# simon-donike/NIR-GAN

Hardware: AMD Instinct MI355X
Metric: 256x256 RGB tiles/sec (G+D fwd+bwd+step) (higher is better)
Workload: dtype f32 (3xbf16 split, 6 products, f32 accumulate) for the contractions with 32-channel runs incl. the Winograd plane GEMMs; exact f32 MFMA for the first / last layers; f32 everywhere else; 1 GPU; configs[1]: 6-block ResnetGenerator + 3-layer PatchGAN, bs=16/GPU, 256x256, GAN+L1, padding=0, fp32-equivalent MFMA (three bf16 terms, six products); global_batch=16, parallelism=dp1

## Files before the change

### include/nirgan_hip.h

```cpp
#ifndef NIRGAN_HIP_H
#define NIRGAN_HIP_H

#include <stdint.h>

#ifdef __cplusplus
extern "C" {
#endif

#define NIRGAN_MAX_TAPS 16

#define NIRGAN_OK 0
#define NIRGAN_ERR_ARG (-1)
#define NIRGAN_ERR_LAUNCH (-2)

#define NIRGAN_ACT_NONE 0
#define NIRGAN_ACT_RELU 1
#define NIRGAN_ACT_LRELU 2
#define NIRGAN_ACT_TANH 3

#define NIRGAN_BORDER_KEEP 0
#define NIRGAN_BORDER_REFLECT 1

int nirgan_version(void);
const char* nirgan_last_error(void);

typedef struct {
    const float* in;  int64_t in_elems;
    int in_hp, in_wp, in_cs;
    int run;
    int in_stride, in_oh, in_ow;
    int ntaps;
    int tap_dh[NIRGAN_MAX_TAPS], tap_dw[NIRGAN_MAX_TAPS];
    const float* w;   int64_t w_elems;
    const float* bias;
    float* out;       int64_t out_elems;
    int out_hp, out_wp, out_cs;
    int out_stride, out_oh, out_ow;
    int B, OH, OW, N;
    const float* zero_page;
    int ksplit; float* split_ws; int64_t split_ws_elems;
    int precision;
    int w_bf16;
    int in_bf16;
    float* stats_ws; int64_t stats_ws_elems; int stats_chunk0, stats_chunks;
    const float* fuse_y; const float* fuse_mean; const float* fuse_rstd;
    int fuse_h, fuse_w, fuse_oh, fuse_ow, fuse_act; float fuse_slope;
    float* fuse_part; int64_t fuse_part_elems; int fuse_chunk0, fuse_chunks;
    int out_bf16, fuse_y_bf16;
    int algo;
    const void* w_x3; int64_t w_x3_plane;
    int out_span;
} nirgan_conv_desc;
#define NIRGAN_CONV_TILE128 1
#define NIRGAN_CONV_X3_R4 4

int nirgan_conv_igemm(const nirgan_conv_desc* d, void* stream);

typedef struct {
    const float* p;   int64_t p_elems;
    int p_hp, p_wp, p_cs, p_oh, p_ow;
    const float* q;   int64_t q_elems;
    int q_hp, q_wp, q_cs, q_stride, q_oh, q_ow;
    int run, ntaps;
    int tap_dh[NIRGAN_MAX_TAPS], tap_dw[NIRGAN_MAX_TAPS];
    int B, OH, OW, N;
    float* slabs;     int64_t slab_elems;
    int nsplit, rows_per_split;
    const float* zero_page;
    int precision;
    int nplanes; int64_t p_plane, q_plane;
    int pq_bf16;
    int algo;
} nirgan_wgrad_desc;
#define NIRGAN_WGRAD_ONE_UNIT 1
#define NIRGAN_WGRAD_TILE128 2

int nirgan_wgrad_igemm(const nirgan_wgrad_desc* d, void* stream);

int nirgan_conv_igemm_group(const nirgan_conv_desc* const* descs, int n, void* stream);

int nirgan_conv_wgrad_pair(const nirgan_conv_desc* c, const nirgan_wgrad_desc* w, void* stream);

const char* nirgan_conv_kernel_name(const nirgan_conv_desc* d);
const char* nirgan_wgrad_kernel_name(const nirgan_wgrad_desc* d);
const char* nirgan_conv_wgrad_pair_kernel_name(const nirgan_conv_desc* c, const nirgan_wgrad_desc* w);

int nirgan_reduce_rows(const float* slabs, int nsplit, int N, int K, const int32_t* map,
                       float* dst, int64_t dst_elems, int dst_row_stride, int accumulate, void* stream);
int nirgan_reduce_rows_part(const float* slabs, int nsplit, int N, int row0, int rows, int K, const int32_t* map,
                            float* dst, int64_t dst_elems, int dst_row_stride, int accumulate, void* stream);

int nirgan_reduce_rows_batch(const int64_t* jobs_device, int njobs, int total_blocks, void* stream);

int nirgan_pack_rows(const float* src, int64_t src_elems, int src_row_stride, const int32_t* map,
                     float* dst, int N, int K, void* stream);

int nirgan_pack_rows_bf16(const float* src, int64_t src_elems, int src_row_stride, const int32_t* map,
                          void* dst_bf16, int N, int K, void* stream);
int nirgan_pack_rows_batch(const int64_t* jobs_device, int njobs, int total_blocks, void* stream);

int nirgan_split3(const float* src, void* dst_bf16, int64_t n, int64_t plane, void* stream);

typedef struct {
    const float* y;
    int B, H, W, C;
    int norm; float eps;
    float* mean; float* rstd;
    int act; float slope;
    const float* residual; int r_hp, r_wp, r_pad;
    float* out; int o_hp, o_wp, o_pad; int border;
    float* ws; int64_t ws_elems;
    void* out_bf16;
    int stats_chunks;
    const float* stats_shift;
    int y_bf16;
} nirgan_in_fwd_desc;

int64_t nirgan_instnorm_ws_elems(int B, int H, int W, int C);
int nirgan_instnorm_fwd(const nirgan_in_fwd_desc* d, void* stream);

typedef struct {
    const float* g; int g_hp, g_wp, g_pad, g_fold;
    const float* g2;
    const float* a; int a_hp, a_wp, a_pad;
    int act; float slope;
    const float* y; const float* mean; const float* rstd; int norm;
    int B, H, W, C;
    float* dy; int d_hp, d_wp, d_pad;
    float* gsum_out;
    float* dbias;
    float* ws; int64_t ws_elems;
    void* dy_bf16;
    int sums_chunks;
// ... 208 lines not shown
int nirgan_location_encoder(const nirgan_locenc_desc* d, void* stream);

typedef struct {
    const float* image; const float* reference;
    int B, N;
    void* ws; int64_t ws_bytes;
    float* out;
} nirgan_hist_match_desc;

int64_t nirgan_hist_match_ws_bytes(int B, int N);
int nirgan_hist_match(const nirgan_hist_match_desc* d, void* stream);

typedef struct {
    const float* dy; int dy_hp, dy_wp, dy_pad;
    int B, H, W, K;
    float* Yt; int64_t Yt_elems;
    int r;
} nirgan_wino_dy_desc;

typedef struct {
    const float* x; int x_hp, x_wp;
    int B, H, W, C, K;
    const float* U; const float* bias;
    float* V; int64_t V_elems;
    float* M; int64_t M_elems;
    float* y;
    const float* zero_page;
    int r;
    float* stats_ws; int64_t stats_ws_elems;
    const float* fuse_y; const float* fuse_mean; const float* fuse_rstd; const float* fuse_g2;
    float* fuse_gz; float* fuse_part; int64_t fuse_part_elems; int fuse_act; float fuse_slope;
    int algo;
    const void* U3;
} nirgan_wino6_desc;
#define NIRGAN_W6_ONE_TILE 1
#define NIRGAN_W6_DIRECT_TILE 3
#define NIRGAN_W6_X3_R4 5
#define NIRGAN_W6_PATCH_PER_THREAD 16
#define NIRGAN_W6_PATCH_PER_LANES 17
const char* nirgan_wino6_gemm_kernel_name(const nirgan_wino6_desc* d);
const char* nirgan_wino6_pair_kernel_name(const nirgan_wino6_desc* d, const nirgan_wgrad_desc* w);

int64_t nirgan_wino6_tiles(int B, int H, int W);
int64_t nirgan_wino6_tiles_r(int B, int H, int W, int r);
int nirgan_wino6_weights(const float* w, int K, int C, int transpose_flip, float* U, void* stream);
int nirgan_wino6_weights_r(const float* w, int K, int C, int r, int transpose_flip, float* U, void* stream);
int nirgan_wino6_weights_x3(const float* w, int K, int C, int r, int transpose_flip, float* U, void* U3_bf16, void* stream);
int nirgan_wino6_weights_batch(const int64_t* jobs_device, int njobs, int total_blocks, void* stream);
int nirgan_wino6_input(const nirgan_wino6_desc* d, void* stream);
int nirgan_wino6_input_norm(const nirgan_wino6_desc* d, const float* y, const float* mean, const float* rstd, int act, float slope, void* stream);
int nirgan_wino6_gemm(const nirgan_wino6_desc* d, void* stream);
int nirgan_wino6_gemm_wgrad_pair(const nirgan_wino6_desc* c, const nirgan_wgrad_desc* w, void* stream);
int nirgan_wino6_output(const nirgan_wino6_desc* d, void* stream);
int nirgan_wino6_conv3x3(const nirgan_wino6_desc* d, void* stream);
int nirgan_wino6_dy(const nirgan_wino_dy_desc* d, void* stream);
int nirgan_wino6_input_dy(const nirgan_wino6_desc* c, const nirgan_wino_dy_desc* y, void* stream);
int nirgan_wino6_input_dy_norm(const nirgan_wino6_desc* c, const nirgan_wino_dy_desc* y, const nirgan_in_bwd_desc* n, void* stream);
int nirgan_wino6_wgrad_finish(const float* slabs, int nsplit, int K, int C, float* grad, int accumulate, void* stream);
int nirgan_wino6_wgrad_finish_r(const float* slabs, int nsplit, int K, int C, int r, float* grad, int accumulate, void* stream);
int nirgan_wino6_wgrad_finish_batch(const float* const* slabs, float* const* grads, int n, int nsplit, int K, int C, int r, int accumulate, void* stream);

int nirgan_bilinear_fwd(const float* src, int B, int SH, int SW, float* dst, int OH, int OW, void* stream);
int nirgan_bilinear_bwd(const float* ddst, int B, int OH, int OW, float* dsrc, int SH, int SW, void* stream);

typedef struct {
    const float* z; const float* e; const float* scale;
    int style;
    int B, H, W, C;
    float* out; int o_hp, o_wp, o_pad;
} nirgan_inject_fwd_desc;
int nirgan_inject_fwd(const nirgan_inject_fwd_desc* d, void* stream);

typedef struct {
    const float* g; const float* a; int a_hp, a_wp, a_pad;
    const float* z; const float* e; const float* scale;
    int style;
    int B, H, W, C;
    float* dz; float* de; float* dscale;
    float* ws; int64_t ws_elems;
} nirgan_inject_bwd_desc;
int nirgan_inject_bwd(const nirgan_inject_bwd_desc* d, void* stream);

int nirgan_colsum(const float* x, int64_t rows, int cols, float* out, int accumulate, void* stream);

int nirgan_param_scale_fwd(const float* x, const float* param, float* out, int64_t n, void* stream);
int nirgan_param_scale_bwd(const float* gout, const float* x, const float* param, float* gx, float* dparam, float* ws, int64_t ws_elems,
                           int64_t n, void* stream);
int nirgan_fill(float* dst, int64_t n, float value, void* stream);
int nirgan_axpy(float* y, const float* x, int64_t n, float alpha, void* stream);

#define NIRGAN_OP_CONV 1
#define NIRGAN_OP_WGRAD 2
#define NIRGAN_OP_IN_FWD 3
#define NIRGAN_OP_IN_BWD 4
typedef struct { int op; const void* desc; } nirgan_plan_entry;
int nirgan_run_plan(const nirgan_plan_entry* entries, int n, void* stream);

int64_t nirgan_tile_count(int B, int H, int W, int tile, int margin);
int nirgan_tile_gather(const float* scene, int B, int C, int H, int W, int tile, int margin, int first, int n, float* tiles, void* stream);
int nirgan_tile_scatter(const float* tiles, int B, int C, int H, int W, int tile, int margin, int first, int n, float* scene, void* stream);

#define NIRGAN_BLEND_LINEAR 0
#define NIRGAN_BLEND_COSINE 1
typedef struct {
    int B, C, H, W;
    int tile, margin, overlap;
    int window;
    int first, n;
    float* scene;
    float* tiles;
} nirgan_tile_blend_desc;
int64_t nirgan_tile_count_ov(int B, int H, int W, int tile, int margin, int overlap);
int nirgan_tile_gather_ov(const nirgan_tile_blend_desc* d, void* stream);
int nirgan_tile_blend(const nirgan_tile_blend_desc* d, void* stream);

typedef struct {
    int n, C, H, W;
    int views;
    const float* src;
    float* dst;
} nirgan_tile_views_desc;
int nirgan_tile_views_expand(const nirgan_tile_views_desc* d, void* stream);
int nirgan_tile_views_merge(const nirgan_tile_views_desc* d, void* stream);

#define NIRGAN_GEO_SLAB_MAX 2048
typedef struct {
    const double* points;
    int n_points;
    int n_verts;
    const double* verts;
    const int32_t* ring_start;
    const int32_t* ring_region;
    int n_rings, n_regions;
    double* region_box;
    const int32_t* ring_start_host;
    const int32_t* ring_region_host;
    int slab_verts;
    uint32_t* ws;
    int64_t ws_bytes;
    int32_t* region;
} nirgan_point_regions_desc;
int64_t nirgan_point_regions_ws_bytes(int n_points, int n_regions);
int nirgan_region_boxes(const nirgan_point_regions_desc* d, void* stream);
int nirgan_point_regions(const nirgan_point_regions_desc* d, void* stream);

#define NIRGAN_RASTER_U8 0
#define NIRGAN_RASTER_I16 1
#define NIRGAN_RASTER_I32 2
typedef struct {
    const double* points;
    int n_points;
    int H, W, dtype;
    const void* raster;
    double x0, dx, y0, dy;
    int has_nodata, nodata;
    int32_t* value;
} nirgan_raster_lookup_desc;
int nirgan_raster_lookup(const nirgan_raster_lookup_desc* d, void* stream);

#ifdef __cplusplus
}
#endif
#endif
```

### nir-gan_amd/csrc/elementwise.hip

```cpp
#include "common.h"

namespace {

inline int grid_for(int64_t total, int cap = 4096) {
    const int64_t g = (total + 255) / 256;
    return int(g < cap ? (g < 1 ? 1 : g) : cap);
}

__global__ __launch_bounds__(256) void adam_kernel(float* __restrict__ p, const float* __restrict__ g, float* __restrict__ m,
                                                   float* __restrict__ v, int64_t n, float b1, float b2, float eps,
                                                   float step_size, float inv_sqrt_bc2) {
    const int64_t n4 = n >> 2;
    for (int64_t i = blockIdx.x * int64_t(blockDim.x) + threadIdx.x; i < n4; i += int64_t(gridDim.x) * blockDim.x) {
        f32x4 pp = reinterpret_cast<f32x4*>(p)[i];
        const f32x4 gg = reinterpret_cast<const f32x4*>(g)[i];
        f32x4 mm = reinterpret_cast<f32x4*>(m)[i], vv = reinterpret_cast<f32x4*>(v)[i];
#pragma unroll
        for (int k = 0; k < 4; ++k) {
            mm[k] = mm[k] * b1 + (1.f - b1) * gg[k];
            vv[k] = vv[k] * b2 + (1.f - b2) * gg[k] * gg[k];
            const float denom = sqrtf(vv[k]) * inv_sqrt_bc2 + eps;
            pp[k] -= step_size * (mm[k] / denom);
        }
        reinterpret_cast<f32x4*>(p)[i] = pp;
// ... 65 lines not shown
            }
        }
        ds[i] = acc;
    }
}

struct InjP {
    const float* z; const float* e; const float* scale; int style;
    int HW, W, C;
    float* out; int o_row, o_img, o_org;
    const float* g; const float* a; int a_row, a_img, a_org;
    float* dz; float* de; float* dscale; float* ws;
};

__global__ __launch_bounds__(256) void inject_fwd_kernel(const InjP p, int64_t npix) {
    const int q4 = p.C / 4;
    const float s = p.scale ? p.scale[0] : 1.f;
    const int64_t total = npix * q4;
    for (int64_t i = blockIdx.x * int64_t(blockDim.x) + threadIdx.x; i < total; i += int64_t(gridDim.x) * blockDim.x) {
        const int q = int(i % q4);
        const int64_t pix = i / q4;
        const int b = int(pix / p.HW), r = int(pix - int64_t(b) * p.HW);
        const int h = r / p.W, w = r - h * p.W;
        const float ev = p.e[pix];
        f32x4 v = *reinterpret_cast<const f32x4*>(p.z + pix * p.C + q * 4);
        if (p.style == 0) v = v * (p.scale ? 1.f + s * ev : ev); else v = v + s * ev;
#pragma unroll
        for (int k = 0; k < 4; ++k) v[k] = v[k] > 0.f ? v[k] : 0.f;
        *reinterpret_cast<f32x4*>(p.out + int64_t(b) * p.o_img + p.o_org + int64_t(h) * p.o_row + int64_t(w) * p.C + q * 4) = v;
    }
}

__global__ __launch_bounds__(256) void inject_bwd_kernel(const InjP p, int64_t npix) {
    __shared__ float red[256];
    const int q4 = p.C / 4 < 256 ? p.C / 4 : 256;
    const int ppi = 256 / q4;
    const int tid = threadIdx.x, q = tid % q4, pl = tid / q4;
    const float s = p.scale ? p.scale[0] : 1.f;
    float ds_acc = 0.f;
    for (int64_t base = int64_t(blockIdx.x) * ppi; base < npix; base += int64_t(gridDim.x) * ppi) {
        const int64_t pix = base + pl;
        float de_part = 0.f;
        if (pl < ppi && pix < npix) {
            const int b = int(pix / p.HW), r = int(pix - int64_t(b) * p.HW);
            const int h = r / p.W, w = r - h * p.W;
            const float ev = p.e[pix];
            const float mul = p.scale ? 1.f + s * ev : ev;
            for (int qq = q; qq < p.C / 4; qq += q4) {
                const f32x4 gv = *reinterpret_cast<const f32x4*>(p.g + pix * p.C + qq * 4);
                const f32x4 av = *reinterpret_cast<const f32x4*>(p.a + int64_t(b) * p.a_img + p.a_org + int64_t(h) * p.a_row + int64_t(w) * p.C + qq * 4);
                const f32x4 zv = *reinterpret_cast<const f32x4*>(p.z + pix * p.C + qq * 4);
                f32x4 gm, dz;
#pragma unroll
                for (int k = 0; k < 4; ++k) {
                    gm[k] = av[k] > 0.f ? gv[k] : 0.f;
                    if (p.style == 0) {
                        dz[k] = gm[k] * mul;
                        de_part += gm[k] * zv[k] * s;
                        ds_acc += gm[k] * zv[k] * ev;
                    } else {
                        dz[k] = gm[k];
                        de_part += gm[k] * s;
                        ds_acc += gm[k] * ev;
                    }
                }
                *reinterpret_cast<f32x4*>(p.dz + pix * p.C + qq * 4) = dz;
            }
        }
        red[tid] = de_part;
        __syncthreads();
        if (q == 0 && pl < ppi && pix < npix) {
            float t = 0.f;
            for (int k = 0; k < q4; ++k) t += red[pl * q4 + k];
            p.de[pix] = t;
        }
        __syncthreads();
    }
    ds_acc = ng_wave_sum(ds_acc);
    if ((tid & 63) == 0) red[tid >> 6] = ds_acc;
    __syncthreads();
    if (tid == 0 && p.dscale) p.ws[blockIdx.x] = (red[0] + red[1]) + (red[2] + red[3]);
}

__global__ __launch_bounds__(1024) void colsum_kernel(const float* __restrict__ x, int64_t rows, int cols, float* __restrict__ out, int accumulate) {
    __shared__ float red[16][64];
    const int cl = threadIdx.x & 63, c = blockIdx.x * 64 + cl, rl = threadIdx.x >> 6;
    float s0 = 0.f, s1 = 0.f, s2 = 0.f, s3 = 0.f;
    if (c < cols) {
        int64_t r = rl;
        for (; r + 48 < rows; r += 64) {
            s0 += x[r * cols + c];
            s1 += x[(r + 16) * cols + c];
            s2 += x[(r + 32) * cols + c];
            s3 += x[(r + 48) * cols + c];
        }
        for (; r < rows; r += 16) s0 += x[r * cols + c];
    }
    red[rl][cl] = (s0 + s1) + (s2 + s3);
    __syncthreads();
    if (rl == 0 && c < cols) {
        float t = 0.f;
#pragma unroll
        for (int i = 0; i < 16; ++i) t += red[i][cl];
        out[c] = accumulate ? out[c] + t : t;
    }
}

__global__ void fill_kernel(float* __restrict__ dst, int64_t n, float v) {
    for (int64_t i = blockIdx.x * int64_t(blockDim.x) + threadIdx.x; i < n; i += int64_t(gridDim.x) * blockDim.x) dst[i] = v;
}

__global__ void axpy_kernel(float* __restrict__ y, const float* __restrict__ x, int64_t n, float a) {
    for (int64_t i = blockIdx.x * int64_t(blockDim.x) + threadIdx.x; i < n; i += int64_t(gridDim.x) * blockDim.x) y[i] += a * x[i];
}


__global__ __launch_bounds__(256) void param_scale_fwd_kernel(const float* __restrict__ x, const float* __restrict__ param, float* __restrict__ out, int64_t n) {
    const float c = *param;
    for (int64_t i = blockIdx.x * 256ll + threadIdx.x; i < n; i += int64_t(gridDim.x) * 256) out[i] = x[i] * c;
}
__global__ __launch_bounds__(256) void param_scale_bwd_kernel(const float* __restrict__ gout, const float* __restrict__ x, const float* __restrict__ param,
                                                               float* __restrict__ gx, float* __restrict__ ws, int64_t n) {
    __shared__ float red[4];
    const float c = *param;
    float acc = 0.f;
    for (int64_t i = blockIdx.x * 256ll + threadIdx.x; i < n; i += int64_t(gridDim.x) * 256) {
        const float g = gout[i];
        gx[i] = g * c;
        acc += g * x[i];
    }
    acc = ng_wave_sum(acc);
    if ((threadIdx.x & 63) == 0) red[threadIdx.x >> 6] = acc;
    __syncthreads();
    if (threadIdx.x == 0) ws[blockIdx.x] = (red[0] + red[1]) + (red[2] + red[3]);
}

__global__ __launch_bounds__(256) void partials_finish_kernel(const float* __restrict__ ws, int rows, int nv, float* dst) {
    __shared__ float part[4][8];
    const int tid = threadIdx.x, lane = tid & 63, wave = tid >> 6;
    float acc[8] = {0, 0, 0, 0, 0, 0, 0, 0};
    for (int r = tid; r < rows; r += 256)
        for (int i = 0; i < nv; ++i) acc[i] += ws[size_t(r) * nv + i];
    for (int i = 0; i < nv; ++i) {
        const float v = ng_wave_sum(acc[i]);
        if (lane == 0) part[wave][i] = v;
    }
    __syncthreads();
    if (tid < nv) atomicAdd(dst + tid, (part[0][tid] + part[1][tid]) + (part[2][tid] + part[3][tid]));
}

}

int ng_partials_finish(const float* ws, int rows, int nv, float* dst, hipStream_t st) {
    NG_REQUIRE(ws && dst && rows > 0 && nv > 0 && nv <= 8, "partials_finish: bad arguments");
    hipLaunchKernelGGL(partials_finish_kernel, dim3(1), dim3(256), 0, st, ws, rows, nv, dst);
    return nirgan_check_launch("partials_finish");
}

extern "C" int nirgan_adam(float* p, const float* g, float* m, float* v, int64_t n, float lr, float beta1, float beta2,
                           float eps, int step, void* stream) {
    NG_REQUIRE(p && g && m && v && n > 0 && step >= 1, "adam: bad arguments");
    NG_REQUIRE(ng_aligned16(p) && ng_aligned16(g) && ng_aligned16(m) && ng_aligned16(v), "adam: pointers must be 16-byte aligned");
    const double bc1 = 1.0 - pow(double(beta1), double(step));
    const double bc2 = 1.0 - pow(double(beta2), double(step));
    const float step_size = float(double(lr) / bc1);
    const float inv_sqrt_bc2 = float(1.0 / sqrt(bc2));
    hipLaunchKernelGGL(adam_kernel, dim3(grid_for((n + 3) / 4, 2048)), dim3(256), 0, static_cast<hipStream_t>(stream),
                       p, g, m, v, n, beta1, beta2, eps, step_size, inv_sqrt_bc2);
    return nirgan_check_launch("adam");
}

extern "C" int nirgan_bilinear_fwd(const float* src, int B, int SH, int SW, float* dst, int OH, int OW, void* stream) {
    NG_REQUIRE(src && dst && B > 0 && SH > 0 && SW > 0 && OH > 0 && OW > 0, "bilinear_fwd: bad arguments");
    hipLaunchKernelGGL(bilinear_fwd_kernel, dim3(grid_for(int64_t(B) * OH * OW)), dim3(256), 0, static_cast<hipStream_t>(stream), src, B, SH, SW, dst, OH, OW);
    return nirgan_check_launch("bilinear_fwd");
}

extern "C" int nirgan_bilinear_bwd(const float* ddst, int B, int OH, int OW, float* dsrc, int SH, int SW, void* stream) {
    NG_REQUIRE(ddst && dsrc && B > 0 && SH > 0 && SW > 0 && OH > 0 && OW > 0, "bilinear_bwd: bad arguments");
    hipStream_t st = static_cast<hipStream_t>(stream);
    hipLaunchKernelGGL(bilinear_bwd_kernel, dim3(grid_for(int64_t(B) * SH * SW)), dim3(256), 0, st, ddst, B, OH, OW, dsrc, SH, SW);
    return nirgan_check_launch("bilinear_bwd");
}

extern "C" int nirgan_inject_fwd(const nirgan_inject_fwd_desc* d, void* stream) {
    NG_REQUIRE(d && d->z && d->e && d->out, "inject_fwd: null pointer");
    NG_REQUIRE(d->B > 0 && d->H > 0 && d->W > 0 && d->C >= 4 && d->C % 4 == 0, "inject_fwd: bad shape");
    NG_REQUIRE(d->o_hp == d->H + 2 * d->o_pad && d->o_wp == d->W + 2 * d->o_pad, "inject_fwd: output geometry mismatch");
    InjP p = {};
    p.z = d->z; p.e = d->e; p.scale = d->scale; p.style = d->style; p.HW = d->H * d->W; p.W = d->W; p.C = d->C;
    p.out = d->out; p.o_row = d->o_wp * d->C; p.o_img = d->o_hp * p.o_row; p.o_org = d->o_pad * p.o_row + d->o_pad * d->C;
    const int64_t npix = int64_t(d->B) * p.HW;
    hipLaunchKernelGGL(inject_fwd_kernel, dim3(grid_for(npix * (d->C / 4))), dim3(256), 0, static_cast<hipStream_t>(stream), p, npix);
    return nirgan_check_launch("inject_fwd");
}

extern "C" int nirgan_inject_bwd(const nirgan_inject_bwd_desc* d, void* stream) {
    NG_REQUIRE(d && d->g && d->a && d->z && d->e && d->dz && d->de, "inject_bwd: null pointer");
    NG_REQUIRE(d->B > 0 && d->H > 0 && d->W > 0 && d->C >= 4 && d->C % 4 == 0, "inject_bwd: bad shape");
    NG_REQUIRE(d->a_hp == d->H + 2 * d->a_pad && d->a_wp == d->W + 2 * d->a_pad, "inject_bwd: mask geometry mismatch");
    InjP p = {};
    p.z = d->z; p.e = d->e; p.scale = d->scale; p.style = d->style; p.HW = d->H * d->W; p.W = d->W; p.C = d->C;
    p.g = d->g; p.a = d->a; p.a_row = d->a_wp * d->C; p.a_img = d->a_hp * p.a_row; p.a_org = d->a_pad * p.a_row + d->a_pad * d->C;
    p.dz = d->dz; p.de = d->de; p.dscale = d->dscale;
    const int64_t npix = int64_t(d->B) * p.HW;
    const int q4 = d->C / 4 < 256 ? d->C / 4 : 256;
    const int ppi = 256 / q4;
    int64_t g = (npix + ppi - 1) / ppi;
    g = g < 2048 ? g : 2048;
    NG_REQUIRE(!d->dscale || (d->ws && d->ws_elems >= g), "inject_bwd: dscale needs a workspace of %lld floats (block partial sums, fixed-order finish)", (long long)g);
    p.ws = d->ws;
    hipLaunchKernelGGL(inject_bwd_kernel, dim3(int(g)), dim3(256), 0, static_cast<hipStream_t>(stream), p, npix);
    if (d->dscale) return ng_partials_finish(d->ws, int(g), 1, d->dscale, static_cast<hipStream_t>(stream));
    return nirgan_check_launch("inject_bwd");
}

extern "C" int nirgan_param_scale_fwd(const float* x, const float* param, float* out, int64_t n, void* stream) {
    NG_REQUIRE(x && param && out && n > 0, "param_scale_fwd: bad arguments");
    hipLaunchKernelGGL(param_scale_fwd_kernel, dim3(grid_for(n)), dim3(256), 0, static_cast<hipStream_t>(stream), x, param, out, n);
    return nirgan_check_launch("param_scale_fwd");
}

extern "C" int nirgan_param_scale_bwd(const float* gout, const float* x, const float* param, float* gx, float* dparam, float* ws, int64_t ws_elems,
                                      int64_t n, void* stream) {
    NG_REQUIRE(gout && x && param && gx && dparam && ws && n > 0, "param_scale_bwd: bad arguments");
    int64_t g = (n + 255) / 256;
    g = g < 1024 ? g : 1024;
    NG_REQUIRE(ws_elems >= g, "param_scale_bwd: workspace holds %lld floats, %lld needed", (long long)ws_elems, (long long)g);
    hipLaunchKernelGGL(param_scale_bwd_kernel, dim3(int(g)), dim3(256), 0, static_cast<hipStream_t>(stream), gout, x, param, gx, ws, n);
    return ng_partials_finish(ws, int(g), 1, dparam, static_cast<hipStream_t>(stream));
}

extern "C" int nirgan_colsum(const float* x, int64_t rows, int cols, float* out, int accumulate, void* stream) {
    NG_REQUIRE(x && out && rows > 0 && cols > 0, "colsum: bad arguments");
    hipLaunchKernelGGL(colsum_kernel, dim3((cols + 63) / 64), dim3(1024), 0, static_cast<hipStream_t>(stream), x, rows, cols, out, accumulate);
    return nirgan_check_launch("colsum");
}

extern "C" int nirgan_fill(float* dst, int64_t n, float value, void* stream) {
    NG_REQUIRE(dst && n > 0, "fill: bad arguments");
    hipLaunchKernelGGL(fill_kernel, dim3(grid_for(n)), dim3(256), 0, static_cast<hipStream_t>(stream), dst, n, value);
    return nirgan_check_launch("fill");
}

extern "C" int nirgan_axpy(float* y, const float* x, int64_t n, float alpha, void* stream) {
    NG_REQUIRE(y && x && n > 0, "axpy: bad arguments");
    hipLaunchKernelGGL(axpy_kernel, dim3(grid_for(n)), dim3(256), 0, static_cast<hipStream_t>(stream), y, x, n, alpha);
    return nirgan_check_launch("axpy");
}

extern "C" int nirgan_run_plan(const nirgan_plan_entry* entries, int n, void* stream) {
    NG_REQUIRE(entries || n == 0, "run_plan: null entries");
    for (int i = 0; i < n; ++i) {
        int rc;
        switch (entries[i].op) {
            case NIRGAN_OP_CONV: rc = nirgan_conv_igemm(static_cast<const nirgan_conv_desc*>(entries[i].desc), stream); break;
            case NIRGAN_OP_WGRAD: rc = nirgan_wgrad_igemm(static_cast<const nirgan_wgrad_desc*>(entries[i].desc), stream); break;
            case NIRGAN_OP_IN_FWD: rc = nirgan_instnorm_fwd(static_cast<const nirgan_in_fwd_desc*>(entries[i].desc), stream); break;
            case NIRGAN_OP_IN_BWD: rc = nirgan_instnorm_bwd(static_cast<const nirgan_in_bwd_desc*>(entries[i].desc), stream); break;
            default: nirgan_set_error("run_plan: unknown op %d at entry %d", entries[i].op, i); return NIRGAN_ERR_ARG;
        }
        if (rc != NIRGAN_OK) return rc;
    }
    return NIRGAN_OK;
}
```

### nir-gan_amd/csrc/igemm_conv.hip

```cpp
#include "igemm_tiles.h"
#include "igemm_tile256.h"
#include "igemm_x3.h"
#include <cstdlib>
#include "igemm_x3r.h"

namespace {

template <int BN, int PREC = 0, bool WB16 = false, bool AB16 = false>
__global__ __launch_bounds__(256, 2) void conv_igemm_kernel(const ng::ConvParams p) {
    __shared__ __attribute__((aligned(16))) char st0[(128 + BN) * 128];
    __shared__ __attribute__((aligned(16))) char st1[(128 + BN) * 128];
    ng::conv_tile<BN, PREC, WB16, AB16>(p, blockIdx.x, st0, st1);
}

__global__ __launch_bounds__(512, 2) void conv_igemm256_kernel(const ng::ConvParams p) {
    __shared__ __attribute__((aligned(16))) char lds[ng::T256_LDS];
    ng::conv_tile256(p, ng_xcd_remap(blockIdx.x, gridDim.x), lds);
}

template <int BN>
__global__ __launch_bounds__(512, 2) void conv_x3_kernel(const ng::X3Work w) {
    __shared__ __attribute__((aligned(16))) char sA0[ng::X3_A_BYTES];
    __shared__ __attribute__((aligned(16))) char sA1[ng::X3_A_BYTES];
    __shared__ __attribute__((aligned(16))) char sB0[3 * BN * 64];
// ... 47 lines not shown
__global__ __launch_bounds__(256, 2) void conv_group_kernel(const ConvGroup g) {
    __shared__ __attribute__((aligned(16))) char st0[(128 + BN) * 128];
    __shared__ __attribute__((aligned(16))) char st1[(128 + BN) * 128];
    const int bid = blockIdx.x;
    int k = 0;
    if (bid >= g.first[1]) k = 1;
    if (bid >= g.first[2]) k = 2;
    if (bid >= g.first[3]) k = 3;
    if (k == 0) ng::conv_tile<BN, PREC, WB16, AB16>(g.p[0], bid, st0, st1);
    else if (k == 1) ng::conv_tile<BN, PREC, WB16, AB16>(g.p[1], bid - g.first[1], st0, st1);
    else if (k == 2) ng::conv_tile<BN, PREC, WB16, AB16>(g.p[2], bid - g.first[2], st0, st1);
    else ng::conv_tile<BN, PREC, WB16, AB16>(g.p[3], bid - g.first[3], st0, st1);
}

}

int ng::ng_cu_count_conv() {
    static int cus = 0;
    if (cus == 0) {
        int dev = 0, n = 0;
        if (hipGetDevice(&dev) != hipSuccess || hipDeviceGetAttribute(&n, hipDeviceAttributeMultiprocessorCount, dev) != hipSuccess || n <= 0) n = 256;
        cus = n;
#ifdef NG_X3R_STAMP
        if (const char* e = getenv("NG_X3R_CUS")) cus = atoi(e);
#endif
    }
    return cus;
}
using ng::ng_cu_count_conv;

int ng::ng_launch_conv_x3(const ng::ConvParams* ps, const int n, const int bn, const int nplanes, const long long in_plane, const long long w3_pstride,
                          const long long out_plane, hipStream_t st, const char* what) {
    ng::X3Work w;
    int total = 0;
    for (int i = 0; i < n; ++i) { w.p[i] = ps[i]; w.first[i] = total; total += ng::conv_x3_tiles(ps[i], bn) * (nplanes > 1 ? nplanes : 1); }
    for (int i = n; i < 4; ++i) { w.p[i] = ps[0]; w.first[i] = 0x7fffffff; }
    w.first[n] = total;
    for (int i = n + 1; i < 5; ++i) w.first[i] = 0x7fffffff;
    w.n = n;
    w.nplanes = nplanes > 1 ? nplanes : 1;
    w.in_plane = in_plane; w.w3_pstride = w3_pstride; w.out_plane = out_plane;
    w.spread = 0;
    for (int i = 0; i < 4; ++i) w.start[i] = 0;
    const int G = ng_cu_count_conv();
    bool unequal = false;
    for (int i = 1; i < n; ++i) unequal = unequal || ps[i].K != ps[0].K;
    if (n >= 2 && w.nplanes == 1 && unequal && total >= G && G <= 1024) {
        long long load[2 * 1024 + 1];
        for (int i = 0; i < G; ++i) load[i] = 0;
        int order[4] = {0, 1, 2, 3};
        for (int i = 0; i < n; ++i)
            for (int j = i + 1; j < n; ++j)
                if (ps[order[j]].K > ps[order[i]].K) { const int t = order[i]; order[i] = order[j]; order[j] = t; }
        for (int oi = 0; oi < n; ++oi) {
            const int k = order[oi];
            const int rem = (w.first[k + 1] - w.first[k]) % G;
            if (rem == 0) continue;
            const long long cost = ps[k].K / 32 + 3;
            long long prefix[2 * 1024 + 1];
            prefix[0] = 0;
            for (int i = 0; i < 2 * G; ++i) prefix[i + 1] = prefix[i] + load[i % G];
            int best = 0;
            for (int s0 = 1; s0 < G; ++s0)
                if (prefix[s0 + rem] - prefix[s0] < prefix[best + rem] - prefix[best]) best = s0;
            for (int t = 0; t < rem; ++t) load[(best + t) % G] += cost;
            w.start[k] = best;
        }
        w.spread = 1;
    }
    const dim3 grid(total < G ? total : G);
    switch (ng::conv_x3_route(ps, n, bn)) {
        case ng::X3R_GENERIC: hipLaunchKernelGGL((conv_x3r_kernel<128, 2>), grid, dim3(256), 0, st, w); break;
        case ng::X3R_STATS: hipLaunchKernelGGL((conv_x3r_kernel<128, 1>), grid, dim3(256), 0, st, w); break;
        case ng::X3R_PLAIN: hipLaunchKernelGGL((conv_x3r_kernel<128, 0>), grid, dim3(256), 0, st, w); break;
        case ng::X3_N128: hipLaunchKernelGGL(conv_x3_kernel<128>, grid, dim3(512), 0, st, w); break;
        case ng::X3_N64: hipLaunchKernelGGL(conv_x3_kernel<64>, grid, dim3(512), 0, st, w); break;
    }
    return nirgan_check_launch(what);
}

ng::X3Kernel ng::conv_x3_route(const ng::ConvParams* ps, const int n, const int bn) {
    bool reg_fed = true, gen = false, stats = false;
    for (int i = 0; i < n; ++i) {
        reg_fed = reg_fed && ng::conv_x3r_ok(ps[i], bn);
        gen = gen || ng::conv_x3r_generic(ps[i]);
        stats = stats || ng::conv_x3r_stats(ps[i]);
    }
    if (reg_fed) return gen ? ng::X3R_GENERIC : (stats ? ng::X3R_STATS : ng::X3R_PLAIN);
    return bn == 128 ? ng::X3_N128 : ng::X3_N64;
}

enum ConvKernel { CONV_K_X3R, CONV_K_X3_N128, CONV_K_X3_N64, CONV_K_TILE256, CONV_K_TILE128, CONV_K_TILE64 };
static const char* const CONV_KERNEL_NAMES[] = {"conv_x3r_kernel<128>", "conv_x3_kernel<128>", "conv_x3_kernel<64>", "conv_igemm256_kernel",
                                                "conv_igemm_kernel<128>", "conv_igemm_kernel<64>"};
struct ConvRoute { ConvKernel k; int bn; };
static ConvRoute conv_route(const ng::ConvParams* ps, const int n, const bool group) {
    bool x3 = ps[0].prec == 3;
    for (int i = 0; i < n; ++i) x3 = x3 && ng::conv_x3_ok(ps[i]) && (ps[i].N % 128 == 0) == (ps[0].N % 128 == 0);
    if (x3) {
        const int bn = ng::conv_x3_bn(ps, n, ng_cu_count_conv());
        const ng::X3Kernel k = ng::conv_x3_route(ps, n, bn);
        return {k == ng::X3_N128 ? CONV_K_X3_N128 : (k == ng::X3_N64 ? CONV_K_X3_N64 : CONV_K_X3R), bn};
    }
    if (!group && ps[0].algo != NIRGAN_CONV_TILE128 && ng::conv_tile256_ok(ps[0])) return {CONV_K_TILE256, 0};
    return {ps[0].N > 64 ? CONV_K_TILE128 : CONV_K_TILE64, 0};
}
static bool conv_route_x3(const ConvRoute& r) { return r.k == CONV_K_X3R || r.k == CONV_K_X3_N128 || r.k == CONV_K_X3_N64; }

#ifdef NG_X3R_STAMP
extern "C" int nirgan_x3r_stamps(unsigned long long* host, int n) {
    return hipMemcpyFromSymbol(host, HIP_SYMBOL(ng::ng_x3r_stamps), size_t(n) * 8) == hipSuccess ? 0 : -1;
}
#endif

extern "C" int nirgan_split3(const float* src, void* dst_bf16, int64_t n, int64_t plane, void* stream) {
    NG_REQUIRE(src && dst_bf16 && n > 0 && n % 8 == 0 && plane >= n && plane % 8 == 0, "split3: n and plane must be positive multiples of 8, plane >= n");
    NG_REQUIRE(ng_aligned16(src) && ng_aligned16(dst_bf16), "split3: pointers must be 16-byte aligned");
    hipLaunchKernelGGL(split3_kernel, dim3((unsigned)((n / 8 + 255) / 256)), dim3(256), 0, static_cast<hipStream_t>(stream),
                       src, static_cast<unsigned short*>(dst_bf16), (long long)n, (long long)plane);
    return nirgan_check_launch("split3");
}

extern "C" int nirgan_conv_igemm(const nirgan_conv_desc* d, void* stream) {
    ng::ConvParams p;
    const int rc = ng::build_conv_params(d, p);
    if (rc != NIRGAN_OK) return rc;
    hipStream_t st = static_cast<hipStream_t>(stream);
    const ConvRoute r = conv_route(&p, 1, false);
    if (conv_route_x3(r)) return ng::ng_launch_conv_x3(&p, 1, r.bn, 1, 0, 0, 0, st, "conv_igemm (three-term split tile)");
    if (p.prec == 3) {
        NG_REQUIRE(p.ch == p.N, "conv: out_span = 2 needs a problem the three-term split tile covers (run %% 32 == 0, N %% 64 == 0)");
        p.prec = 0;
    }
    if (r.k == CONV_K_TILE256) {
        hipLaunchKernelGGL(conv_igemm256_kernel, dim3(((p.M + 255) >> 8) * (p.N >> 8)), dim3(512), 0, st, p);
        return nirgan_check_launch("conv_igemm (256 x 256 tile)");
    }
    const dim3 grid(p.mtiles * p.ntiles * p.ksplit);
    ng::conv_tile_form(p, [&](auto form) {
        using F = decltype(form);
        if (r.k == CONV_K_TILE128) hipLaunchKernelGGL((conv_igemm_kernel<128, F::prec, F::wb16, F::ab16>), grid, dim3(256), 0, st, p);
        else hipLaunchKernelGGL((conv_igemm_kernel<64, F::prec, F::wb16, F::ab16>), grid, dim3(256), 0, st, p);
    });
    if (p.ksplit > 1) {
        const long long total = (long long)p.M * (p.N / 4);
        const int grid = int((total + 255) / 256 < 4096 ? (total + 255) / 256 : 4096);
        hipLaunchKernelGGL(conv_splitk_reduce_kernel, dim3(grid), dim3(256), 0, st, p);
    }
    return nirgan_check_launch("conv_igemm");
}

extern "C" const char* nirgan_conv_kernel_name(const nirgan_conv_desc* d) {
    ng::ConvParams p;
    if (ng::build_conv_params(d, p) != NIRGAN_OK) return nullptr;
    return CONV_KERNEL_NAMES[conv_route(&p, 1, false).k];
}

extern "C" int nirgan_conv_igemm_group(const nirgan_conv_desc* const* descs, int n, void* stream) {
    NG_REQUIRE(descs != nullptr && n >= 1 && n <= 4, "conv_igemm_group: 1..4 descriptors");
    ConvGroup g;
    int total = 0;
    bool wide = false;
    for (int i = 0; i < n; ++i) {
        NG_REQUIRE(descs[i] != nullptr, "conv_igemm_group: null descriptor %d", i);
        const int rc = ng::build_conv_params(descs[i], g.p[i]);
        if (rc != NIRGAN_OK) return rc;
        NG_REQUIRE(descs[i]->ksplit <= 1, "conv_igemm_group: split-K descriptors are not groupable");
// ... 27 lines not shown
```

### nir-gan_amd/csrc/igemm_tiles.h

```cpp
#pragma once
#include <type_traits>
#include "common.h"

#ifdef NG_DIAG
__device__ __forceinline__ unsigned long long ng_stamp() {
    unsigned long long t;
    __builtin_amdgcn_sched_barrier(0);
    asm volatile("s_memtime %0\n\ts_waitcnt lgkmcnt(0)" : "=s"(t) :: "memory");
    __builtin_amdgcn_sched_barrier(0);
    return t;
}
#define NG_DIAG_ENTRY const unsigned long long ng_entry = ng_stamp();
#define NG_DIAG_DECL unsigned long long ng_t0 = ng_stamp(), ng_a = ng_t0, ng_wait = 0, ng_body = 0, ng_b = 0;
#define NG_WAIT_BEGIN ng_a = ng_stamp();
#define NG_WAIT_END ng_b = ng_stamp(); ng_wait += ng_b - ng_a; ng_a = ng_b;
#define NG_BODY_END ng_b = ng_stamp(); ng_body += ng_b - ng_a; ng_a = ng_b;
#define NG_DIAG_STORE(dbg, blk)                                                                          \
    if ((threadIdx.x & 63) == 0 && (dbg) != nullptr) {                                                     \
        unsigned long long* o = (dbg) + (size_t(blk) * 4 + (threadIdx.x >> 6)) * 6;                         \
        const unsigned long long te = ng_stamp();                                                           \
        o[0] = ng_t0; o[1] = ng_loop_end; o[2] = te; o[3] = ng_wait; o[4] = ng_body;                        \
        o[5] = ng_t0 - ng_entry;                               \
    }
#else
#define NG_DIAG_ENTRY
#define NG_DIAG_DECL
#define NG_WAIT_BEGIN
#define NG_WAIT_END
#define NG_BODY_END
#define NG_DIAG_STORE(dbg, blk)
#endif

namespace ng {

typedef __bf16 bf16x8 __attribute__((ext_vector_type(8)));
typedef float f32x8 __attribute__((ext_vector_type(8)));

__device__ __forceinline__ bf16x8 ng_bf16_round(const f32x8 v) { return __builtin_convertvector(v, bf16x8); }
__device__ __forceinline__ f32x8 ng_bf16_widen(const bf16x8 v) { return __builtin_convertvector(v, f32x8); }

template <int PREC>
__device__ __forceinline__ void ng_mfma_bf16(const f32x8 a, const f32x8 b, f32x16& acc) {
    const bf16x8 ah = ng_bf16_round(a), bh = ng_bf16_round(b);
    if constexpr (PREC == 2) {
        const bf16x8 am = ng_bf16_round(a - ng_bf16_widen(ah)), bm = ng_bf16_round(b - ng_bf16_widen(bh));
        acc = __builtin_amdgcn_mfma_f32_32x32x16_bf16(am, bh, acc, 0, 0, 0);
        acc = __builtin_amdgcn_mfma_f32_32x32x16_bf16(ah, bm, acc, 0, 0, 0);
    }
    acc = __builtin_amdgcn_mfma_f32_32x32x16_bf16(ah, bh, acc, 0, 0, 0);
}

struct ConvParams {
    const float* in;
    const float* w;
    const float* bias;
    float* out;
    const float* zero;
    int in_row, in_img, in_cs, run, in_stride, in_org;
    int ntaps;
    int tap_off[NIRGAN_MAX_TAPS];
    int K;
    int out_cs, out_row, out_img, out_stride, out_org;
    int OW, OHW, M, N;
    int mtiles, ntiles;
    int ksplit;
    float* split_ws;
    unsigned long long* dbg;
    int w_bf16;
    int in_bf16;
    int prec;
    float* stats;
    int stats_chunk0, stats_cps;
    const float* f_y; const float* f_mean; const float* f_rstd; float* f_part;
    int f_img, f_row, f_org, f_act, f_chunk0, f_cps;
    float f_slope;
    int out16, f_y16;
    int algo;
    int off32;
    const unsigned short* w3;
    long long w3_plane;
    int ch;
    long long out_elems;
};


template <int BN, int PREC, bool WB16 = false, bool AB16 = false>
__device__ __forceinline__ void conv_tile(const ConvParams& p, const int block_id, char* st0, char* st1,
                                          const float* in_base = nullptr, const float* w_base = nullptr, float* out_base = nullptr) {
    NG_DIAG_ENTRY
    const float* const p_in = in_base ? in_base : p.in;
    const float* const p_w = w_base ? w_base : p.w;
    float* const p_out = out_base ? out_base : p.out;
    static_assert(!WB16 || PREC == 1, "bf16-stored weights are consumed by the bf16 operand mode only");
    static_assert(!AB16 || WB16, "bf16 activations come with bf16-stored weights");
    constexpr int BM = 128;
    constexpr int A_BYTES = BM * 128;
    constexpr int B_BYTES = BN * 128;
    constexpr int STAGE = A_BYTES + B_BYTES;
    constexpr int NT = BN / 64;
    constexpr int BI = BN / 32;
    constexpr bool WIDE = AB16;
    constexpr int KS = WIDE ? 64 : 32;

    const int tid = threadIdx.x, lane = tid & 63;
    const int wave = __builtin_amdgcn_readfirstlane(tid >> 6);
    const int tiles = p.mtiles * p.ntiles;
    const int rid = ng_xcd_remap(block_id, tiles * p.ksplit);
    const int ksp = rid / tiles, id = rid - ksp * tiles;
    const int n0 = (id % p.ntiles) * BN, m0 = (id / p.ntiles) * BM;

    const int lrow = lane >> 3, lchunk = lane & 7;
    constexpr int AIW = 4;
    int a_base[AIW], a_col[AIW];
#pragma unroll
    for (int i = 0; i < AIW; ++i) {
        const int row = (wave * 4 + i) * 8 + lrow;
        const int lc = lchunk ^ ((row >> 1) & 7);
        const int cw = AB16 ? 8 : 4;
        int m = m0 + row;
        m = m < p.M ? m : p.M - 1;
        const int b = m / p.OHW, r = m - b * p.OHW;
        const int oh = r / p.OW, ow = r - oh * p.OW;
        a_col[i] = lc * cw;
        a_base[i] = b * p.in_img + oh * p.in_stride * p.in_row + ow * p.in_stride * p.in_cs + p.in_org + lc * cw;
    }
    constexpr int BIW = (WB16 && !WIDE) ? BN / 64 : BI;
    int b_base[BIW], b_col[BIW];
    bool b_ok[BIW];
#pragma unroll
    for (int i = 0; i < BIW; ++i) {
        if constexpr (WIDE) {
            const int row = (wave * BI + i) * 8 + lrow;
            const int lc = lchunk ^ ((row >> 1) & 7);
            const int n = n0 + row;
            b_ok[i] = n < p.N;
            b_col[i] = lc * 8;
            b_base[i] = (b_ok[i] ? n : 0) * p.K + lc * 8;
        } else if constexpr (WB16) {
            const int row = (wave * BIW + i) * 16 + (lane >> 2);
            const int lc = (lane & 3) ^ ((row >> 2) & 3);
            const int n = n0 + row;
            b_ok[i] = n < p.N;
            b_col[i] = lc * 8;
            b_base[i] = (b_ok[i] ? n : 0) * p.K + lc * 8;
        } else {
            const int row = (wave * BI + i) * 8 + lrow;
            const int lc = lchunk ^ ((row >> 1) & 7);
            const int n = n0 + row;
            b_ok[i] = n < p.N;
            b_col[i] = lc * 4;
            b_base[i] = (b_ok[i] ? n : 0) * p.K + lc * 4;
        }
    }

    constexpr int ESA = AB16 ? 2 : 4, ESB = WB16 ? 2 : 4;
    unsigned a_boff[AIW], b_boff[BIW];
#pragma unroll
    for (int i = 0; i < AIW; ++i) a_boff[i] = unsigned(a_base[i]) * unsigned(ESA);
#pragma unroll
    for (int i = 0; i < BIW; ++i) b_boff[i] = unsigned(b_base[i]) * unsigned(ESB);
    const bool inside = p.off32 != 0;

    auto issue = [&](char* sA, int t, int c0) {
        char* sB = sA + A_BYTES;
        const int toff = p.tap_off[t] + c0;
// ... 210 lines not shown
    }

#ifdef NG_DIAG
    const unsigned long long ng_loop_end = ng_stamp();
#endif
#ifdef NG_DIAG_SKIP_EPILOGUE
    if (p.dbg == nullptr) {
        float keep = 0.f;
#pragma unroll
        for (int mt = 0; mt < 2; ++mt)
#pragma unroll
            for (int nt = 0; nt < NT; ++nt)
#pragma unroll
                for (int r = 0; r < 16; ++r) keep += acc[mt][nt][r];
        if (keep == 123456.789f) p_out[0] = keep;
        return;
    }
#endif
    if (p.stats != nullptr) {
        const int b = m0 / p.OHW;
        const int chunk = p.stats_chunk0 + ((m0 - b * p.OHW) >> 7) * 2 + wr;
        float* sp = p.stats + (size_t(b) * p.stats_cps + chunk) * 4 * p.N;
#pragma unroll
        for (int nt = 0; nt < NT; ++nt) {
            const float own = acc[0][nt][0], other = __shfl_xor(own, 32, 64);
            const float k = half == 0 ? own : other;
            float s1 = 0.f, s2 = 0.f;
#pragma unroll
            for (int mt = 0; mt < 2; ++mt)
#pragma unroll
                for (int r = 0; r < 16; ++r) {
                    const float v = acc[mt][nt][r] - k;
                    s1 += v;
                    s2 += v * v;
                }
            s1 += __shfl_xor(s1, 32, 64);
            s2 += __shfl_xor(s2, 32, 64);
            const int col = n0 + wc * (BN / 2) + nt * 32 + (lane & 31);
            if (half == 0 && col < p.N) {
                sp[col] = k;
                sp[p.N + col] = s1;
                sp[2 * p.N + col] = s2;
                sp[3 * p.N + col] = 64.f;
            }
        }
    }
    __syncthreads();
    {
        float* half_base = reinterpret_cast<float*>(wr == 0 ? st0 : st1);
#pragma unroll
        for (int mt = 0; mt < 2; ++mt)
#pragma unroll
            for (int nt = 0; nt < NT; ++nt) {
                const int col = wc * (BN / 2) + nt * 32 + (lane & 31);
#pragma unroll
                for (int r = 0; r < 16; ++r) {
                    const int row_l = mt * 32 + (r & 3) + 8 * (r >> 2) + 4 * half;
                    half_base[row_l * BN + col] = acc[mt][nt][r];
                }
            }
    }
    __syncthreads();
    auto write_out = [&](auto wtag) {
        constexpr int W = decltype(wtag)::value;
        constexpr int LPR = BN / W;
        constexpr int RPP = 256 / LPR;
        typedef float fW __attribute__((ext_vector_type(W)));
        typedef __bf16 bW __attribute__((ext_vector_type(W)));
        const int chunk = tid % LPR, row0 = tid / LPR;
        const int n = n0 + chunk * W;
        fW bv = {};
        const bool to_ws = p.ksplit > 1;
        if (p.bias != nullptr && !to_ws) {
#pragma unroll
            for (int j = 0; j < W; ++j) bv[j] = n + j < p.N ? p.bias[n + j] : 0.f;
        }
        int m = m0 + row0;
        const int mc = m < p.M ? m : p.M - 1;
        int b = mc / p.OHW;
        const int r0 = mc - b * p.OHW;
        int oh = r0 / p.OW, ow = r0 - oh * p.OW;
        const int OH = p.OHW / p.OW;
        const bool fused = p.f_y != nullptr;
        const int fb = m0 / p.OHW;
        fW fm = {}, fr = {}, s1 = {}, s2 = {};
        if (fused && n < p.N) {
            fm = *reinterpret_cast<const fW*>(p.f_mean + size_t(fb) * p.N + n);
            fr = *reinterpret_cast<const fW*>(p.f_rstd + size_t(fb) * p.N + n);
        }
        const float fneg = p.f_act == NIRGAN_ACT_RELU ? 0.f : (p.f_act == NIRGAN_ACT_LRELU ? p.f_slope : 1.f);
#pragma unroll 4
        for (int row = row0; row < BM; row += RPP) {
            if (m < p.M && n < p.N) {
                const float* src = reinterpret_cast<const float*>(row < 64 ? st0 : st1) + (row & 63) * BN + chunk * W;
                fW v = *reinterpret_cast<const fW*>(src);
                v += bv;
                const int oidx = b * p.out_img + oh * p.out_stride * p.out_row + ow * p.out_stride * p.out_cs + p.out_org + n;
                float* dst = to_ws ? p.split_ws + ((size_t(ksp) * p.M + m) * p.N + n) : p_out + oidx;
                if constexpr (W == 8) {
                    *reinterpret_cast<bW*>(reinterpret_cast<unsigned short*>(p_out) + oidx) = __builtin_convertvector(v, bW);
                } else if (p.out16) {
                    *reinterpret_cast<bW*>(reinterpret_cast<unsigned short*>(p_out) + oidx) = __builtin_convertvector(v, bW);
                } else if (n + 4 <= p.N) {
                    *reinterpret_cast<fW*>(dst) = v;
                } else {
#pragma unroll
                    for (int j = 0; j < W; ++j)
                        if (n + j < p.N) dst[j] = v[j];
                }
                if (fused) {
                    const size_t yidx = size_t(b) * p.f_img + size_t(oh * p.out_stride) * p.f_row + size_t(ow * p.out_stride) * p.N + p.f_org + n;
                    fW y4;
                    if (p.f_y16) y4 = __builtin_convertvector(*reinterpret_cast<const bW*>(reinterpret_cast<const unsigned short*>(p.f_y) + yidx), fW);
                    else y4 = *reinterpret_cast<const fW*>(p.f_y + yidx);
                    const fW z = (y4 - fm) * fr;
#pragma unroll
                    for (int j = 0; j < W; ++j) {
                        const float gz = z[j] > 0.f ? v[j] : v[j] * fneg;
                        s1[j] += gz;
                        s2[j] += gz * z[j];
                    }
                }
            }
            m += RPP;
            ow += RPP;
            while (ow >= p.OW) { ow -= p.OW; ++oh; }
            while (oh >= OH) { oh -= OH; ++b; }
        }
        if (fused) {
            __syncthreads();
            fW* red = reinterpret_cast<fW*>(st0);
            red[tid * 2] = s1;
            red[tid * 2 + 1] = s2;
            __syncthreads();
            if (tid < LPR && n < p.N) {
                fW t1 = {}, t2 = {};
#pragma unroll 4
                for (int r = 0; r < RPP; ++r) {
                    t1 += red[(r * LPR + tid) * 2];
                    t2 += red[(r * LPR + tid) * 2 + 1];
                }
                float* pp = p.f_part + (size_t(fb) * p.f_cps + p.f_chunk0 + ((m0 - fb * p.OHW) >> 7)) * 2 * p.N + n;
                *reinterpret_cast<fW*>(pp) = t1;
                *reinterpret_cast<fW*>(pp + p.N) = t2;
            }
        }
    };
    if (p.out16 && p.N % BN == 0 && p.ksplit <= 1 && ((p.out_cs | p.out_org | p.out_row | p.out_img) & 7) == 0) write_out(std::integral_constant<int, 8>{});
    else write_out(std::integral_constant<int, 4>{});
    NG_DIAG_STORE(p.dbg, block_id)
}

struct WgradParams {
    const float* p;
    const float* q;
    float* slabs;
    const float* zero;
    int p_row, p_img, p_cs, p_org;
    int q_row, q_img, q_cs, q_stride, q_org;
    int run, ntaps;
    int tap_off[NIRGAN_MAX_TAPS];
    int K, OW, OH, OHW, M, N;
    int rows_per_split, nsplit, ntiles_n, ntiles_k;
    int prec;
    int pq_bf16;
    int nplanes;
    long long p_plane, q_plane;
    unsigned long long* dbg;
    int fast32_bytes;
    int fast32;
};


template <int TN, int PREC>
__device__ __forceinline__ void wgrad_tile(const WgradParams& p, const int block_id, char* st0, char* st1) {
    constexpr int P_BYTES = 32 * TN * 4;
    constexpr int Q_BYTES = 32 * 128 * 4;
    constexpr int STAGE = P_BYTES + Q_BYTES;
    constexpr int LPR = TN / 4;
    constexpr int RPI = 64 / LPR;
    constexpr int PI = TN / 32;
    constexpr int EA = TN / 64;

    const int tid = threadIdx.x, lane = tid & 63;
    const int wave = __builtin_amdgcn_readfirstlane(tid >> 6);
    const int tiles = p.ntiles_n * p.ntiles_k;
    const int per_plane = tiles * p.nsplit;
    const int rid = ng_xcd_remap(block_id, per_plane * p.nplanes);
    const int plane = rid / per_plane, id = rid - plane * per_plane;
    const int split = id / tiles, tile = id - split * tiles;
    const int n0 = (tile % p.ntiles_n) * TN, j0 = (tile / p.ntiles_n) * 128;
    const int mstart = split * p.rows_per_split;
    int mend = mstart + p.rows_per_split;
    mend = mend < p.M ? mend : p.M;
    const int nk = mend > mstart ? (mend - mstart + 31) >> 5 : 0;
// ... 605 lines not shown
template <int P, bool WB, bool AB> struct TileForm { static constexpr int prec = P; static constexpr bool wb16 = WB, ab16 = AB; };
template <class F> inline void conv_tile_form(const ConvParams& p, F&& f) {
    if (p.prec == 0) f(TileForm<0, false, false>{});
    else if (p.prec == 1 && p.in_bf16) f(TileForm<1, true, true>{});
    else if (p.prec == 1 && p.w_bf16) f(TileForm<1, true, false>{});
    else if (p.prec == 1) f(TileForm<1, false, false>{});
    else f(TileForm<2, false, false>{});
}

inline int build_conv_params(const nirgan_conv_desc* d, ConvParams& p) {
    NG_REQUIRE(d != nullptr, "conv: null descriptor");
    NG_REQUIRE(d->in && d->w && d->out && d->zero_page, "conv: null pointer");
    NG_REQUIRE(ng_aligned16(d->in) && ng_aligned16(d->w) && ng_aligned16(d->zero_page) && ng_aligned16(d->out), "conv: in/w/out/zero_page must be 16-byte aligned");
    NG_REQUIRE(d->out_cs % 4 == 0 || d->N < 4, "conv: out_cs must be a multiple of 4");
    NG_REQUIRE(d->B > 0 && d->OH > 0 && d->OW > 0 && d->N > 0, "conv: empty problem B=%d OH=%d OW=%d N=%d", d->B, d->OH, d->OW, d->N);
    NG_REQUIRE(d->ntaps >= 1 && d->ntaps <= NIRGAN_MAX_TAPS, "conv: ntaps=%d out of range", d->ntaps);
    NG_REQUIRE(d->run > 0 && d->run % 4 == 0 && d->in_cs > 0 && d->in_cs % 4 == 0, "conv: run=%d and in_cs=%d must be positive multiples of 4", d->run, d->in_cs);
    NG_REQUIRE(d->in_stride >= 1 && d->out_stride >= 1, "conv: strides must be >= 1");
    NG_REQUIRE(d->in_elems < (int64_t(1) << 31) && d->out_elems < (int64_t(1) << 31) && d->w_elems < (int64_t(1) << 31), "conv: buffers must be < 2^31 floats");
    NG_REQUIRE(d->in_elems >= int64_t(d->B) * d->in_hp * d->in_wp * d->in_cs, "conv: in_elems too small");
    NG_REQUIRE(d->out_elems >= int64_t(d->B) * d->out_hp * d->out_wp * d->out_cs, "conv: out_elems too small");
    NG_REQUIRE(d->w_elems >= int64_t(d->N) * d->ntaps * d->run, "conv: w_elems too small");
    const int span = d->out_span > 1 ? d->out_span : 1;
    const bool span_view = span == 2 && d->out_cs == d->N;
    NG_REQUIRE(span == 1 || (span == 2 && d->precision == 3 && d->N % 8 == 0 && (span_view ? d->fuse_y == nullptr : (d->out_cs == d->N / 2 && d->out_stride >= 2))
                             && !d->out_bf16 && !d->fuse_y_bf16 && d->ksplit <= 1 && d->w_x3 != nullptr),
               "conv: out_span=%d needs precision 3 with its weight planes, out_cs == N / 2 and out_stride >= 2 (or out_cs == N), fp32 tensors and no split-K", d->out_span);
    const int ch = d->N / span;
    NG_REQUIRE(ch <= d->out_cs, "conv: %d channels per pixel exceed out_cs=%d", ch, d->out_cs);
    int dh0 = d->tap_dh[0], dh1 = d->tap_dh[0], dw0 = d->tap_dw[0], dw1 = d->tap_dw[0];
    for (int t = 1; t < d->ntaps; ++t) {
        dh0 = d->tap_dh[t] < dh0 ? d->tap_dh[t] : dh0; dh1 = d->tap_dh[t] > dh1 ? d->tap_dh[t] : dh1;
        dw0 = d->tap_dw[t] < dw0 ? d->tap_dw[t] : dw0; dw1 = d->tap_dw[t] > dw1 ? d->tap_dw[t] : dw1;
    }
    NG_REQUIRE(d->in_oh + dh0 >= 0 && (d->OH - 1) * d->in_stride + d->in_oh + dh1 < d->in_hp, "conv: input rows out of range");
    NG_REQUIRE(d->in_ow + dw0 >= 0 && int64_t((d->OW - 1) * d->in_stride + d->in_ow + dw1) * d->in_cs + d->run <= int64_t(d->in_wp) * d->in_cs, "conv: input columns out of range");
    NG_REQUIRE(d->out_oh >= 0 && (d->OH - 1) * d->out_stride + d->out_oh < d->out_hp && d->out_ow >= 0 && (d->OW - 1) * d->out_stride + d->out_ow + (span_view ? 0 : span - 1) < d->out_wp, "conv: output window out of range");

    p.in = d->in; p.w = d->w; p.bias = d->bias; p.out = d->out; p.zero = d->zero_page;
    p.in_cs = d->in_cs; p.in_row = d->in_wp * d->in_cs; p.in_img = d->in_hp * p.in_row;
    p.run = d->run; p.in_stride = d->in_stride; p.in_org = d->in_oh * p.in_row + d->in_ow * d->in_cs;
    p.ntaps = d->ntaps;
    for (int t = 0; t < NIRGAN_MAX_TAPS; ++t) p.tap_off[t] = t < d->ntaps ? d->tap_dh[t] * p.in_row + d->tap_dw[t] * d->in_cs : 0;
    p.K = d->ntaps * d->run;
    p.out_elems = d->out_elems;
    p.out_cs = d->out_cs; p.out_row = d->out_wp * d->out_cs; p.out_img = d->out_hp * p.out_row;
    p.out_stride = d->out_stride; p.out_org = d->out_oh * p.out_row + d->out_ow * d->out_cs;
    p.OW = d->OW; p.OHW = d->OH * d->OW;
    const int64_t M = int64_t(d->B) * p.OHW;
    NG_REQUIRE(M < (int64_t(1) << 31), "conv: too many output pixels");
    p.M = int(M); p.N = d->N; p.ch = ch;
    p.mtiles = (p.M + 127) / 128;
    p.ntiles = d->N > 64 ? (d->N + 127) / 128 : 1;
    NG_REQUIRE(d->precision >= 0 && d->precision <= 3, "conv: precision=%d (0 fp32, 1 bf16, 2 bf16x3, 3 fp32 as three bf16 terms)", d->precision);
    p.prec = d->precision;
    p.w3 = static_cast<const unsigned short*>(d->w_x3);
    p.w3_plane = d->w_x3_plane;
    NG_REQUIRE(p.w3 == nullptr || (ng_aligned16(p.w3) && d->w_x3_plane >= int64_t(d->N) * d->ntaps * d->run && d->w_x3_plane % 8 == 0), "conv: w_x3 misaligned or w_x3_plane too small");
    p.w_bf16 = d->w_bf16 ? 1 : 0;
    NG_REQUIRE(!p.w_bf16 || (d->precision == 1 && d->run % 8 == 0), "conv: bf16-stored weights need precision 1 and run %% 8 == 0 (run=%d)", d->run);
    p.in_bf16 = d->in_bf16 ? 1 : 0;
    NG_REQUIRE(!p.in_bf16 || (p.w_bf16 && d->in_cs % 8 == 0), "conv: bf16 activations need bf16-stored weights and in_cs %% 8 == 0 (in_cs=%d)", d->in_cs);
    p.off32 = (d->in_elems * (p.in_bf16 ? 2 : 4) < (int64_t(1) << 32) && d->w_elems * (p.w_bf16 ? 2 : 4) < (int64_t(1) << 32)) ? 1 : 0;
    NG_REQUIRE(d->algo == 0 || d->algo == NIRGAN_CONV_TILE128 || d->algo == NIRGAN_CONV_X3_R4,
               "conv: algo=%d (0, NIRGAN_CONV_TILE128 or NIRGAN_CONV_X3_R4)", d->algo);
    p.algo = d->algo;
    p.dbg = nullptr;
    p.ksplit = 1;
    p.split_ws = nullptr;
    p.out16 = d->out_bf16 ? 1 : 0;
    p.f_y16 = d->fuse_y_bf16 ? 1 : 0;
    NG_REQUIRE(!p.out16 || (d->N % 4 == 0 && d->out_cs % 4 == 0 && d->ksplit <= 1), "conv: a bf16 output needs N %% 4 == 0, out_cs %% 4 == 0 and no split-K (N=%d)", d->N);
    p.stats = nullptr; p.stats_chunk0 = 0; p.stats_cps = 0;
    if (d->stats_ws != nullptr) {
        NG_REQUIRE(d->ksplit <= 1 && p.OHW % 128 == 0, "conv: the instance-norm partial sums need OH*OW %% 128 == 0 and no split-K (OH*OW=%d)", p.OHW);
        NG_REQUIRE(d->stats_chunk0 >= 0 && d->stats_chunk0 + p.OHW / 64 * span <= d->stats_chunks, "conv: stats_chunk0 + OH*OW/64 (x out_span) exceeds stats_chunks");
        NG_REQUIRE(d->stats_ws_elems >= int64_t(d->B) * d->stats_chunks * 4 * ch, "conv: stats_ws too small (B * stats_chunks * 4 * channels floats)");
        p.stats = d->stats_ws; p.stats_chunk0 = d->stats_chunk0; p.stats_cps = d->stats_chunks;
    }
    p.f_y = nullptr; p.f_mean = nullptr; p.f_rstd = nullptr; p.f_part = nullptr;
    p.f_img = p.f_row = p.f_org = p.f_chunk0 = p.f_cps = 0; p.f_act = NIRGAN_ACT_NONE; p.f_slope = 0.f;
    if (d->fuse_y != nullptr) {
        NG_REQUIRE(d->ksplit <= 1 && p.OHW % 128 == 0 && d->N % 4 == 0 && d->bias == nullptr, "conv: the fused instance-norm backward sums need OH*OW %% 128 == 0, N %% 4 == 0, no split-K and no bias (OH*OW=%d N=%d)", p.OHW, d->N);
        NG_REQUIRE(d->fuse_mean && d->fuse_rstd && d->fuse_part && ng_aligned16(d->fuse_y) && ng_aligned16(d->fuse_mean) && ng_aligned16(d->fuse_rstd) && ng_aligned16(d->fuse_part), "conv: fuse_mean / fuse_rstd / fuse_part missing or misaligned");
        NG_REQUIRE(d->fuse_oh >= 0 && d->fuse_ow >= 0 && (d->OH - 1) * d->out_stride + d->fuse_oh < d->fuse_h && (d->OW - 1) * d->out_stride + d->fuse_ow + span - 1 < d->fuse_w, "conv: fused window out of y's %d x %d extent", d->fuse_h, d->fuse_w);
        NG_REQUIRE(int64_t(d->B) * d->fuse_h * d->fuse_w * ch < (int64_t(1) << 31), "conv: fuse_y must be < 2^31 floats");
        NG_REQUIRE(d->fuse_chunk0 >= 0 && d->fuse_chunk0 + p.OHW / 128 * span <= d->fuse_chunks, "conv: fuse_chunk0 + OH*OW/128 (x out_span) exceeds fuse_chunks");
        NG_REQUIRE(d->fuse_part_elems >= int64_t(d->B) * d->fuse_chunks * 2 * ch, "conv: fuse_part too small");
        NG_REQUIRE(d->fuse_act == NIRGAN_ACT_NONE || d->fuse_act == NIRGAN_ACT_RELU || d->fuse_act == NIRGAN_ACT_LRELU, "conv: fuse_act=%d", d->fuse_act);
        p.f_y = d->fuse_y; p.f_mean = d->fuse_mean; p.f_rstd = d->fuse_rstd; p.f_part = d->fuse_part;
        p.f_row = d->fuse_w * ch; p.f_img = d->fuse_h * p.f_row; p.f_org = d->fuse_oh * p.f_row + d->fuse_ow * ch;
        p.f_act = d->fuse_act; p.f_slope = d->fuse_slope; p.f_chunk0 = d->fuse_chunk0; p.f_cps = d->fuse_chunks;
    }
    if (d->ksplit > 1) {
        const int nk = d->ntaps * ((d->run + 31) / 32);
        NG_REQUIRE(d->split_ws != nullptr && ng_aligned16(d->split_ws), "conv: split_ws missing or misaligned");
        NG_REQUIRE(d->N % 4 == 0, "conv: split-K needs N %% 4 == 0");
        NG_REQUIRE(d->split_ws_elems >= int64_t(d->ksplit) * M * d->N, "conv: split_ws too small");
        const int per = (nk + d->ksplit - 1) / d->ksplit;
        NG_REQUIRE(per * (d->ksplit - 1) < nk, "conv: ksplit=%d too large for %d K-steps", d->ksplit, nk);
        p.ksplit = d->ksplit;
        p.split_ws = d->split_ws;
    }
    return NIRGAN_OK;
}

inline int build_wgrad_params(const nirgan_wgrad_desc* d, WgradParams& p) {
    NG_REQUIRE(d != nullptr, "wgrad_igemm: null descriptor");
    NG_REQUIRE(d->p && d->q && d->slabs && d->zero_page, "wgrad_igemm: null pointer");
    NG_REQUIRE(ng_aligned16(d->p) && ng_aligned16(d->q) && ng_aligned16(d->slabs) && ng_aligned16(d->zero_page), "wgrad_igemm: pointers must be 16-byte aligned");
    NG_REQUIRE(d->B > 0 && d->OH > 0 && d->OW > 0 && d->N > 0, "wgrad_igemm: empty problem");
    NG_REQUIRE(d->p_cs % 4 == 0 && d->q_cs % 4 == 0 && d->run % 4 == 0 && d->run > 0, "wgrad_igemm: p_cs, q_cs, run must be multiples of 4");
    NG_REQUIRE(d->ntaps >= 1 && d->ntaps <= NIRGAN_MAX_TAPS, "wgrad_igemm: ntaps=%d out of range", d->ntaps);
    NG_REQUIRE(d->q_stride >= 1, "wgrad_igemm: q_stride must be >= 1");
    NG_REQUIRE(d->p_elems < (int64_t(1) << 31) && d->q_elems < (int64_t(1) << 31), "wgrad_igemm: buffers must be < 2^31 floats");
    NG_REQUIRE(d->p_elems >= int64_t(d->B) * d->p_hp * d->p_wp * d->p_cs, "wgrad_igemm: p_elems too small");
    NG_REQUIRE(d->q_elems >= int64_t(d->B) * d->q_hp * d->q_wp * d->q_cs, "wgrad_igemm: q_elems too small");
    NG_REQUIRE(((d->N + 3) & ~3) <= d->p_cs, "wgrad_igemm: N (rounded up to 4) exceeds p_cs");
    NG_REQUIRE(d->p_oh >= 0 && d->OH - 1 + d->p_oh < d->p_hp && d->p_ow >= 0 && d->OW - 1 + d->p_ow < d->p_wp, "wgrad_igemm: p window out of range");
    int dh0 = d->tap_dh[0], dh1 = d->tap_dh[0], dw0 = d->tap_dw[0], dw1 = d->tap_dw[0];
    for (int t = 1; t < d->ntaps; ++t) {
        dh0 = d->tap_dh[t] < dh0 ? d->tap_dh[t] : dh0; dh1 = d->tap_dh[t] > dh1 ? d->tap_dh[t] : dh1;
        dw0 = d->tap_dw[t] < dw0 ? d->tap_dw[t] : dw0; dw1 = d->tap_dw[t] > dw1 ? d->tap_dw[t] : dw1;
    }
    NG_REQUIRE(d->q_oh + dh0 >= 0 && (d->OH - 1) * d->q_stride + d->q_oh + dh1 < d->q_hp, "wgrad_igemm: q rows out of range");
    NG_REQUIRE(d->q_ow + dw0 >= 0 && int64_t((d->OW - 1) * d->q_stride + d->q_ow + dw1) * d->q_cs + d->run <= int64_t(d->q_wp) * d->q_cs, "wgrad_igemm: q columns out of range");
    const int64_t M = int64_t(d->B) * d->OH * d->OW;
    NG_REQUIRE(M < (int64_t(1) << 31), "wgrad_igemm: too many pixels");
    NG_REQUIRE(d->nsplit >= 1 && d->rows_per_split > 0 && d->rows_per_split % 32 == 0 && int64_t(d->nsplit) * d->rows_per_split >= M, "wgrad_igemm: bad split (nsplit=%d rows=%d M=%lld)", d->nsplit, d->rows_per_split, (long long)M);
    const int K = d->ntaps * d->run;
    NG_REQUIRE(d->slab_elems >= int64_t(d->nsplit) * d->N * K, "wgrad_igemm: slab_elems too small");

    p.p = d->p; p.q = d->q; p.slabs = d->slabs; p.zero = d->zero_page;
    p.p_cs = d->p_cs; p.p_row = d->p_wp * d->p_cs; p.p_img = d->p_hp * p.p_row; p.p_org = d->p_oh * p.p_row + d->p_ow * d->p_cs;
    p.q_cs = d->q_cs; p.q_row = d->q_wp * d->q_cs; p.q_img = d->q_hp * p.q_row; p.q_stride = d->q_stride;
    p.q_org = d->q_oh * p.q_row + d->q_ow * d->q_cs;
    p.run = d->run; p.ntaps = d->ntaps;
    for (int t = 0; t < NIRGAN_MAX_TAPS; ++t) p.tap_off[t] = t < d->ntaps ? d->tap_dh[t] * p.q_row + d->tap_dw[t] * d->q_cs : 0;
    p.K = K; p.OW = d->OW; p.OH = d->OH; p.OHW = d->OH * d->OW; p.M = int(M); p.N = d->N;
    p.rows_per_split = d->rows_per_split; p.nsplit = d->nsplit;
    p.ntiles_k = (K + 127) / 128;
    p.ntiles_n = d->N > 64 ? (d->N + 127) / 128 : 1;
    NG_REQUIRE(d->precision >= 0 && d->precision <= 3, "wgrad_igemm: precision=%d (0 fp32, 1 bf16, 2 bf16x3, 3 fp32 as three bf16 terms)", d->precision);
    NG_REQUIRE(d->algo == 0 || d->algo == NIRGAN_WGRAD_ONE_UNIT || d->algo == NIRGAN_WGRAD_TILE128,
               "wgrad_igemm: algo=%d (0, NIRGAN_WGRAD_ONE_UNIT or NIRGAN_WGRAD_TILE128)", d->algo);
    p.prec = d->precision;
    p.nplanes = d->nplanes > 1 ? d->nplanes : 1;
    p.p_plane = d->p_plane; p.q_plane = d->q_plane;
    NG_REQUIRE(p.nplanes == 1 || ((d->precision == 0 || d->precision == 3) && !d->pq_bf16 && d->p_plane > 0 && d->q_plane > 0), "wgrad_igemm: planes need the fp32 tile and positive plane strides");
    NG_REQUIRE(d->slab_elems >= int64_t(p.nplanes) * d->nsplit * d->N * K, "wgrad_igemm: slab_elems too small for %d planes", p.nplanes);
    NG_REQUIRE(d->p_elems >= (p.nplanes - 1) * d->p_plane + int64_t(d->B) * d->p_hp * d->p_wp * d->p_cs && d->q_elems >= (p.nplanes - 1) * d->q_plane + int64_t(d->B) * d->q_hp * d->q_wp * d->q_cs, "wgrad_igemm: p/q too small for the planes");
    p.pq_bf16 = d->pq_bf16 ? 1 : 0;
    p.dbg = nullptr;
    {
        bool taps_ok = true;
        for (int t = 0; t < d->ntaps; ++t) taps_ok = taps_ok && (d->tap_dh[t] * p.q_row + d->tap_dw[t] * d->q_cs >= 0);
        const int ms = d->pq_bf16 ? 64 : 32, es = d->pq_bf16 ? 2 : 4;
        p.fast32_bytes = (d->p_elems * es < (int64_t(1) << 32) && d->q_elems * es < (int64_t(1) << 32)) ? 1 : 0;
        p.fast32 = (taps_ok && d->OW % ms == 0 && p.M % ms == 0 && d->rows_per_split % ms == 0
                    && d->p_elems * es < (int64_t(1) << 32) && d->q_elems * es < (int64_t(1) << 32)) ? 1 : 0;
    }
    NG_REQUIRE(!p.pq_bf16 || (d->precision == 1 && d->N > 64 && d->N % 8 == 0 && d->run % 8 == 0 && d->p_cs % 8 == 0 && d->q_cs % 8 == 0),
               "wgrad_igemm: bf16 twins need precision 1, N > 64 and N, run, p_cs, q_cs multiples of 8");
    return NIRGAN_OK;
}

}
```

### nir-gan_amd/csrc/igemm_x3.h

```cpp
#pragma once
#include "igemm_tiles.h"

namespace ng {

constexpr int X3_A_TERM = 256 * 64;
constexpr int X3_A_BYTES = 3 * X3_A_TERM;

__device__ __forceinline__ int x3_key(const int row) { return (0x78 >> (2 * ((row >> 2) & 3))) & 3; }

__device__ __forceinline__ f32x4 ng_gld16_so(const char* base, unsigned off) {
    asm volatile("" : "+v"(off));
    return *reinterpret_cast<const NG_GLOBAL f32x4*>((const NG_GLOBAL char*)base + off);
}

typedef __bf16 bf16x2 __attribute__((ext_vector_type(2)));
typedef unsigned u32x4 __attribute__((ext_vector_type(4)));
__device__ __forceinline__ unsigned x3_pk(const float a, const float b) {
    const f32x2 v = {a, b};
    return __builtin_bit_cast(unsigned, __builtin_convertvector(v, bf16x2));
}
__device__ __forceinline__ float x3_sub(const float a, const float b) {
    float r;
    asm("v_sub_f32 %0, %1, %2" : "=v"(r) : "v"(a), "v"(b));
    return r;
// ... 187 lines not shown
            X3_RB(bad, 3) X3_WAIT(3) mma(0, A[0], 2); __builtin_amdgcn_sched_barrier(0);
            X3_RA(A[1], aad, 1) X3_WAIT(3) mma(0, A[0], 3); __builtin_amdgcn_sched_barrier(0);
        } else {
            X3_RB(bad, 1) X3_WAIT(3) mma(0, A[0], 0); __builtin_amdgcn_sched_barrier(0);
            X3_RA(A[1], aad, 1) X3_WAIT(3) mma(0, A[0], 1); __builtin_amdgcn_sched_barrier(0);
        }
        X3_RA(A[0], aad, 2) X3_WAIT(3)
#pragma unroll
        for (int nt = 0; nt < NT; ++nt) mma(1, A[1], nt);
        __builtin_amdgcn_sched_barrier(0);
        X3_RA(A[1], aad, 3) X3_WAIT(3)
        mid(0);
#pragma unroll
        for (int nt = 0; nt < NT; ++nt) mma(2, A[0], nt);
        __builtin_amdgcn_sched_barrier(0);
        if constexpr (MORE) { X3_WAIT(3) } else { X3_WAIT(0) }
        mid(1);
#pragma unroll
        for (int nt = 0; nt < NT; ++nt) mma(3, A[1], nt);
    };
#undef X3_WAIT
#undef X3_RB
#undef X3_RA
#undef X3_DSR
    constexpr int ESTORES = 2 * (32 / (64 / (CW / 4)));
    auto step = [&](const int cur, char* nA, char* nB, const bool more, const bool behind_stores = false) {
        if (behind_stores) {
            if constexpr (ESTORES == 16) asm volatile("s_waitcnt vmcnt(16)" ::: "memory");
            else asm volatile("s_waitcnt vmcnt(8)" ::: "memory");
        } else {
            asm volatile("s_waitcnt vmcnt(0)" ::: "memory");
        }
        __syncthreads();
        const unsigned aad = cur == 0 ? a_ad0 : a_ad1, bad = cur == 0 ? b_ad0 : b_ad1;
        if (more) {
            compute(aad, bad, std::true_type{}, [&]() { issueB(nB); loadA(); advance(); }, [&](const int j) { commitA(nA, j); });
        } else {
            compute(aad, bad, std::false_type{}, []() {}, [](const int) {});
        }
    };

    auto epilogue = [&]() -> bool {
        const NG_CONST ConvParams& p = *E.p;
        const int pM = p.M, pN = p.N, OHW = p.OHW, OW = p.OW, OH = p.OHW / p.OW, out_img = p.out_img, out_row = p.out_row * p.out_stride,
                  out_px = p.out_cs * p.out_stride, out_org = p.out_org, f_img = p.f_img, f_row = p.f_row * p.out_stride, f_px = p.ch * p.out_stride,
                  f_org = p.f_org, pC = p.ch, span = p.N / p.ch;
        const float* const f_y = p.f_y;
        const int mbase = E.m0 + wr * 64;
        const bool full = E.m0 + 256 <= pM;
        if (p.stats != nullptr && mbase < pM) {
            const int b = mbase / OHW;
            float* sp = p.stats + (size_t(b) * p.stats_cps + p.stats_chunk0 + ((mbase - b * OHW) >> 6) * span) * 4 * pC;
#pragma unroll
            for (int nt = 0; nt < NT; ++nt) {
                const float k0 = __shfl(acc[0][nt][0], lane & 15, 64);
                float s1 = 0.f, s2 = 0.f;
#pragma unroll
                for (int mt = 0; mt < 4; ++mt)
#pragma unroll
                    for (int r = 0; r < 4; ++r) {
                        const float v = acc[mt][nt][r] - k0;
                        s1 += v;
                        s2 += v * v;
                    }
                s1 += __shfl_xor(s1, 16, 64);
                s2 += __shfl_xor(s2, 16, 64);
                s1 += __shfl_xor(s1, 32, 64);
                s2 += __shfl_xor(s2, 32, 64);
                int col = E.n0 + wc * CW + nt * 16 + (lane & 15);
                if (col >= pC) col += 3 * pC;
                if (lane < 16) {
                    sp[col] = k0;
                    sp[pC + col] = s1;
                    sp[2 * pC + col] = s2;
                    sp[3 * pC + col] = 64.f;
                }
            }
        }
        constexpr int LPR = CW / 4, RPP = 64 / LPR;
        constexpr int SWM = CW / 16 - 1;
        const int sw_wr = ((lane >> 4) & SWM) << 4;
        float* const stg = reinterpret_cast<float*>(wave < 6 ? sA1 + wave * 8192 : sB1 + (wave - 6) * 8192);
        const bool fused = f_y != nullptr;
        const float fneg = p.f_act == NIRGAN_ACT_RELU ? 0.f : (p.f_act == NIRGAN_ACT_LRELU ? p.f_slope : 1.f);
        const int chunk = lane % LPR, lrow = lane / LPR;
        const int n = E.n0 + wc * CW + chunk * 4;
        f32x4 bv = {0.f, 0.f, 0.f, 0.f};
        if (p.bias != nullptr) bv = *reinterpret_cast<const f32x4*>(p.bias + n);
        int m = mbase + lrow;
        const int mc = m < pM ? m : pM - 1;
        int b = mc / OHW;
        const int r0 = mc - b * OHW;
        int oh = r0 / OW, ow = r0 - oh * OW;
        const int fb = (mbase < pM ? mbase : pM - 1) / OHW;
        f32x4 fm = {0.f, 0.f, 0.f, 0.f}, fr = fm, s1 = fm, s2 = fm;
        const int nq = n >= pC ? 1 : 0, nc = n - nq * pC;
        if (fused) {
            fm = *reinterpret_cast<const f32x4*>(p.f_mean + size_t(fb) * pC + nc);
            fr = *reinterpret_cast<const f32x4*>(p.f_rstd + size_t(fb) * pC + nc);
        }
        auto halves = [&](auto full_tag) {
            constexpr bool FULL = decltype(full_tag)::value;
            constexpr int P = 32 / RPP;
#pragma unroll
            for (int h = 0; h < 2; ++h) {
#pragma unroll
                for (int q = 0; q < 2; ++q)
#pragma unroll
                    for (int nt = 0; nt < NT; ++nt)
#pragma unroll
                        for (int r = 0; r < 4; ++r) stg[(q * 16 + (lane >> 4) * 4 + r) * CW + ((nt * 16 + (lane & 15)) ^ sw_wr)] = acc[h * 2 + q][nt][r];
                int ooff[P];
                bool ok[P];
                f32x4 yv[P];
#pragma unroll
                for (int pass = 0; pass < P; ++pass) {
                    ok[pass] = FULL || m < pM;
                    ooff[pass] = b * out_img + oh * out_row + ow * out_px + out_org + n;
                    if (fused && ok[pass]) yv[pass] = *reinterpret_cast<const f32x4*>(f_y + (size_t(b) * f_img + size_t(oh) * f_row + size_t(ow) * f_px + f_org + n));
                    m += RPP;
                    ow += RPP;
                    while (ow >= OW) { ow -= OW; ++oh; }
                    while (oh >= OH) { oh -= OH; ++b; }
                }
#pragma unroll
                for (int pass = 0; pass < P; ++pass) {
                    if (ok[pass]) {
                        f32x4 v = *reinterpret_cast<const f32x4*>(stg + (pass * RPP + lrow) * CW + ((chunk * 4) ^ ((((pass * RPP + lrow) >> 2) & SWM) << 4)));
                        v += bv;
#ifdef NG_X3_NT_STORES
                        __builtin_nontemporal_store(v, reinterpret_cast<f32x4*>(E.out + ooff[pass]));
#else
                        *reinterpret_cast<f32x4*>(E.out + ooff[pass]) = v;
#endif
                        if (fused) {
                            const f32x4 z = (yv[pass] - fm) * fr;
#pragma unroll
                            for (int q = 0; q < 4; ++q) {
                                const float gz = z[q] > 0.f ? v[q] : v[q] * fneg;
                                s1[q] += gz;
                                s2[q] += gz * z[q];
                            }
                        }
                    }
                }
            }
        };
        if (full) halves(std::true_type{}); else halves(std::false_type{});
        if (fused) {
#pragma unroll
            for (int q = 0; q < 4; ++q)
#pragma unroll
                for (int o = LPR; o < 64; o <<= 1) {
                    s1[q] += __shfl_xor(s1[q], o, 64);
                    s2[q] += __shfl_xor(s2[q], o, 64);
                }
            f32x4* const red = reinterpret_cast<f32x4*>(sRed);
            if (lane < LPR) {
                red[(wave * LPR + chunk) * 2] = s1;
                red[(wave * LPR + chunk) * 2 + 1] = s2;
            }
            __syncthreads();
            if ((wr & 1) == 0 && lane < LPR && mbase < pM) {
                const f32x4 t1 = s1 + red[((wave + 2) * LPR + chunk) * 2], t2 = s2 + red[((wave + 2) * LPR + chunk) * 2 + 1];
                float* pp = p.f_part + (size_t(fb) * p.f_cps + p.f_chunk0 + ((mbase - fb * OHW) >> 7) * span + nq) * 2 * pC + nc;
                *reinterpret_cast<f32x4*>(pp) = t1;
                *reinterpret_cast<f32x4*>(pp + pC) = t2;
            }
            __syncthreads();
        }
        return full;
    };

    int item = blockIdx.x;
    if (item >= total) return;
    locate(item, L);
    if (L.nk < 0) return;
    begin();
    loadA();
    issueB(sB0);
    advance();
    commitA(sA0, 0);
    commitA(sA0, 1);
    bool behind = false;
    while (true) {
        zero();
        const int nk = L.nk;
        int k = 0;
        if (nk >= 2) {
            if (behind) step(0, sA1, sB1, true, true); else step(0, sA1, sB1, true);
            step(1, sA0, sB0, 2 < nk);
            k = 2;
        }
        for (; k + 2 <= nk; k += 2) {
            step(0, sA1, sB1, true);
            step(1, sA0, sB0, k + 2 < nk);
        }
        if (k < nk) step(0, sA1, sB1, false);
        E = L;
        item += G;
        bool more = wp->spread ? true : item < total;
        __syncthreads();
        if (more) {
            locate(item, L);
            more = L.nk >= 0;
        }
        if (more) {
            begin();
            loadA();
            issueB(sB0);
            advance();
        }
        behind = epilogue();
        if (!more) break;
        commitA(sA0, 0);
        commitA(sA0, 1);
    }
}
// ... 227 lines not shown
```

### nir-gan_amd/nirgan_hip/engine.py

```python
from __future__ import annotations

import ctypes as C
from typing import Dict, List, Optional

import numpy as np
import torch

from . import geometry as G
from . import lib as L
from .options import OPT

IN_EPS = 1e-5


def _ptr(t: Optional[torch.Tensor]) -> Optional[int]:
    return None if t is None else t.data_ptr()


PRECISIONS = {"fp32": 0, "bf16": 1, "bf16x3": 2}


def precision_code(precision) -> int:
    if precision in PRECISIONS.values():
        return int(precision)
# ... 188 lines not shown
        self.ctx = ctx
        self.cache: Dict[tuple, torch.Tensor] = {}

    def packed(self, plan: Plan, param: torch.Tensor, spec: G.PackSpec, rows_alloc: Optional[int] = None, fp32: bool = False) -> torch.Tensor:
        key = (param.data_ptr(), spec.key, fp32)
        if key in self.cache:
            return self.cache[key]
        rows = max(spec.N, rows_alloc or 0)
        imap = self.ctx.i32(spec.index_map)
        if self.ctx.precision == 1 and spec.run > 0 and spec.run % 8 == 0 and spec.K % 8 == 0 and not fp32:
            buf = torch.zeros(rows, spec.K, dtype=torch.bfloat16, device=self.ctx.device)
            self.ctx.bytes += buf.numel() * 2
            plan.add("nirgan_pack_rows_bf16", param.data_ptr(), param.numel(), spec.row_stride, imap.data_ptr(),
                     buf.data_ptr(), spec.N, spec.K)
        else:
            buf = self.ctx.zeros(rows, spec.K)
            plan.add("nirgan_pack_rows", param.data_ptr(), param.numel(), spec.row_stride, imap.data_ptr(),
                     buf.data_ptr(), spec.N, spec.K)
            if self.ctx.precision == 0 and OPT.split3 and spec.run > 0 and spec.run % 32 == 0 and spec.N % 64 == 0 and not fp32:
                plane = rows * spec.K
                tw = torch.zeros(3 * plane, dtype=torch.bfloat16, device=self.ctx.device)
                self.ctx.bytes += tw.numel() * 2
                self.ctx.keep.append(tw)
                plan.add("nirgan_split3", buf.data_ptr(), tw.data_ptr(), spec.N * spec.K, plane)
                buf.x3 = (tw, plane)
        self.ctx.keep.append(buf)
        self.cache[key] = buf
        return buf

    def packed_pair(self, plan: Plan, param: torch.Tensor, specs: list) -> torch.Tensor:
        a, b = specs
        assert (a.N, a.K, a.run) == (b.N, b.K, b.run) and a.run % 32 == 0 and self.ctx.precision == 0
        key = (param.data_ptr(), "pair", a.key, b.key)
        if key in self.cache:
            return self.cache[key]
        buf = self.ctx.zeros(2 * a.N, a.K)
        plane = 2 * a.N * a.K
        tw = torch.zeros(3 * plane, dtype=torch.bfloat16, device=self.ctx.device)
        self.ctx.bytes += tw.numel() * 2
        for i, spec in enumerate(specs):
            imap = self.ctx.i32(spec.index_map)
            half = buf.data_ptr() + i * a.N * a.K * 4
            plan.add("nirgan_pack_rows", param.data_ptr(), param.numel(), spec.row_stride, imap.data_ptr(), half, spec.N, spec.K)
            plan.add("nirgan_split3", half, tw.data_ptr() + i * a.N * a.K * 2, spec.N * spec.K, plane)
        buf.x3 = (tw, plane)
        self.ctx.keep += [buf, tw]
        self.cache[key] = buf
        return buf

    def doubled(self, plan: Plan, vec: torch.Tensor) -> torch.Tensor:
        key = (vec.data_ptr(), "doubled")
        if key in self.cache:
            return self.cache[key]
        n = vec.numel()
        buf = self.ctx.zeros(2 * n)
        imap = self.ctx.i32(np.concatenate([np.arange(n), np.arange(n)]))
        plan.add("nirgan_pack_rows", vec.data_ptr(), n, 0, imap.data_ptr(), buf.data_ptr(), 1, 2 * n)
        self.ctx.keep.append(buf)
        self.cache[key] = buf
        return buf


def channels_of(d) -> int:
    return d.N // max(1, d.out_span)


class SplitPool:

    def __init__(self, ctx: "Ctx"):
        self.ctx, self.buf = ctx, None

    def get(self, n: int) -> torch.Tensor:
        if self.buf is None or self.buf.numel() < n:
            self.buf = self.ctx.zeros(n)
            self.ctx.keep.append(self.buf)
        return self.buf


def choose_ksplit(tiles: int, nk: int) -> int:
    if tiles >= 400 or nk < 32:
        return 1
    k = max(1, min(8, 1024 // max(tiles, 1), nk // 16))
    return k if k > 1 else 1


def emit_conv(plan: Plan, ctx: Ctx, inp: Halo, taps: G.Taps, w: torch.Tensor, bias, out: Halo, *, N, OH, OW,
              in_stride=1, in_oh=0, in_ow=0, out_stride=1, out_oh=0, out_ow=0, in_hw=None, allow_split=True, out_span=1,
              in_cs=None, out_hw=None, out_cs=None):
    d = L.ConvDesc()
    d.inp, d.in_elems = inp.operand_ptr(d), inp.elems
    if inp.t16 is not None and w.dtype == torch.bfloat16 and taps.run % 8 == 0:
        d.inp, d.in_bf16 = inp.t16.data_ptr(), 1
    d.in_hp, d.in_wp, d.in_cs = (in_hw or (inp.hp, inp.wp)) + (in_cs or inp.C,)
    d.run, d.in_stride, d.in_oh, d.in_ow = taps.run, in_stride, in_oh, in_ow
    _set_taps(d, taps.dh, taps.dw)
    d.w, d.w_elems, d.bias = w.data_ptr(), w.numel(), _ptr(bias)
    d.w_bf16 = 1 if w.dtype == torch.bfloat16 else 0
    if d.w_bf16 and taps.run % 8:
        raise ValueError(f"bf16-stored weights need run % 8 == 0 (run={taps.run})")
    d.out_bf16 = 1 if getattr(out, "is16", False) else 0
    d.out, d.out_elems = (out.ptr_any() if d.out_bf16 else out.ptr), out.elems
    if d.out_bf16:
        allow_split = False
    d.out_hp, d.out_wp, d.out_cs = (out_hw or (out.hp, out.wp)) + (out_cs or out.C,)
    d.out_stride, d.out_oh, d.out_ow = out_stride, out_oh, out_ow
    d.B, d.OH, d.OW, d.N = inp.B, OH, OW, N
    d.zero_page = ctx.zero_page.data_ptr()
    d.precision = ctx.precision
    d.algo = 0 if OPT.tile256 else L.CONV_TILE128
    x3 = getattr(w, "x3", None)
    if (x3 is not None and ctx.precision == 0 and OPT.split3 and taps.run % 32 == 0 and not d.out_bf16 and out.C % 4 == 0
            and (N % 128 == 0 or (N % 64 == 0 and taps.n * taps.run >= 512))):
        d.precision, d.w_x3, d.w_x3_plane = 3, x3[0].data_ptr(), x3[1]
        if OPT.x3_r4:
            d.algo = L.CONV_X3_R4
        allow_split = False
    if out_span > 1:
        assert d.precision == 3 and out.C * out_span == N and (out_stride >= out_span or d.out_cs == N), "out_span needs the three-term split tile and a dense output"
        d.out_span = out_span
    ctx.keep.append(d)
    if plan is not None:
        M = inp.B * OH * OW
        tiles = -(-M // 128) * (-(-N // 128) if N > 64 else 1)
        ks = choose_ksplit(tiles, taps.n * (-(-taps.run // 32))) if (allow_split and N % 4 == 0) else 1
        if ks > 1:
            if not hasattr(ctx, "split_pool"):
                ctx.split_pool = SplitPool(ctx)
            ws = ctx.split_pool.get(ks * M * N)
            d.ksplit, d.split_ws, d.split_ws_elems = ks, ws.data_ptr(), ws.numel()
        plan.add("nirgan_conv_igemm", C.byref(d))
    return d


def emit_wgrad(plan: Plan, ctx: Ctx, p: Halo, q: Halo, taps: G.Taps, spec: G.PackSpec, grad: torch.Tensor, *,
               N, OH, OW, p_oh, p_ow, q_stride=1, q_oh=0, q_ow=0, accumulate=False, slabs_pool=None, pair_with=None):
    K = taps.n * taps.run
    assert K == spec.K, (K, spec.K)
    tiles = (-(-N // 128) if N > 64 else 1) * (-(-K // 128))
    M = p.B * OH * OW
    target = OPT.wgrad_target
    if pair_with is not None:
        c = pair_with
        conv_blocks = -(-(c.B * c.OH * c.OW) // 128) * (-(-c.N // 128) if c.N > 64 else 1)
        total = 512 * max(1, round((conv_blocks + 1024) / 512))
        target = max(total - conv_blocks, 512)
    twins = (ctx.precision == 1 and p.t16 is not None and q.t16 is not None and N > 64 and N % 8 == 0 and taps.run % 8 == 0
             and (pair_with is None or pair_with.in_bf16))
    nsplit, rows = G.wgrad_split(M, tiles, target, 64 if twins else 32)
    x3 = (ctx.precision == 0 and OPT.split3 and N % 128 == 0 and taps.run % 8 == 0 and OW % 32 == 0 and M % 32 == 0
          and all(a * q.wp * q.C + b * q.C >= 0 for a, b in zip(taps.dh, taps.dw)))
    if x3:
        nsplit, rows = G.wgrad_split(M, (N // (256 if N % 256 == 0 else 128)) * (-(-K // 128)), G.CUS, 32)
    if twins and OPT.tile256 and G.wgrad256_ok(M, OH, OW, N, K, taps.run):
        c = pair_with
        fused = c is not None and c.in_bf16 and c.N % 256 == 0 and c.run % 64 == 0 and -(-(c.B * c.OH * c.OW) // 256) * (c.N // 256) >= 128
        nsplit, rows = (G.pair256_plan(M, (N // 256) * (K // 256), -(-(c.B * c.OH * c.OW) // 256) * (c.N // 256), c.ntaps * (c.run // 64)) if fused
                        else G.pair256_plan(M, (N // 256) * (K // 256)))
    need = nsplit * N * K
    deferred = getattr(ctx, "rr_deferred", None)
    slabs = ctx.zeros(need) if deferred is not None else (slabs_pool.get(need) if slabs_pool is not None else ctx.zeros(need))
    ctx.keep.append(slabs)
    d = L.WgradDesc()
    d.p, d.p_elems, d.p_hp, d.p_wp, d.p_cs, d.p_oh, d.p_ow = p.operand_ptr(d), p.elems, p.hp, p.wp, p.C, p_oh, p_ow
    d.q, d.q_elems, d.q_hp, d.q_wp, d.q_cs = q.operand_ptr(d), q.elems, q.hp, q.wp, q.C
    if twins:
        d.p, d.q, d.pq_bf16 = p.t16.data_ptr(), q.t16.data_ptr(), 1
    d.q_stride, d.q_oh, d.q_ow = q_stride, q_oh, q_ow
    d.run = taps.run
    _set_taps(d, taps.dh, taps.dw)
    d.B, d.OH, d.OW, d.N = p.B, OH, OW, N
    d.slabs, d.slab_elems, d.nsplit, d.rows_per_split = slabs.data_ptr(), slabs.numel(), nsplit, rows
    d.zero_page = ctx.zero_page.data_ptr()
    d.precision = 3 if x3 else ctx.precision
    if not OPT.tile256:
        d.algo = L.WGRAD_TILE128
    ctx.keep.append(d)
    imap = ctx.i32(spec.index_map)
    if pair_with is not None:
        plan.add("nirgan_conv_wgrad_pair", C.byref(pair_with), C.byref(d))
    else:
        plan.add("nirgan_wgrad_igemm", C.byref(d))
    if deferred is not None:
        T = taps.n
        conv_layout = (spec.key[:1] == ("cf",) and taps.run % 64 == 0 and T <= 16 and spec.row_stride == taps.run * T and K == T * taps.run)
        deferred.append((slabs, nsplit, N, K, imap, grad, spec.row_stride, 1 if accumulate else 0, T if conv_layout else 0))
        return d
    plan.add("nirgan_reduce_rows", slabs.data_ptr(), nsplit, N, K, imap.data_ptr(), grad.data_ptr(), grad.numel(),
             spec.row_stride, 1 if accumulate else 0)
    return d


def emit_deferred_reduce_rows(plan: Plan, ctx: Ctx, last: bool = True):
    if getattr(ctx, "rr_deferred", None) is None:
        return
    items = ctx.rr_deferred
    ctx.rr_deferred = None if last else []
    for i0 in range(0, len(items), 64):
        part = items[i0:i0 + 64]
        if len(part) == 1:
            slabs, nsplit, N, K, imap, grad, stride, acc, _ = part[0]
            plan.add("nirgan_reduce_rows", slabs.data_ptr(), nsplit, N, K, imap.data_ptr(), grad.data_ptr(), grad.numel(), stride, acc)
            continue
        rows, first = [], 0
        for slabs, nsplit, N, K, imap, grad, stride, acc, T in part:
            rows.append([slabs.data_ptr(), grad.data_ptr(), imap.data_ptr(), nsplit, N, K, grad.numel(), stride | (acc << 32), first, T])
            first += N * ((K // T // 64) if T else ((K + 255) // 256))
        table = torch.tensor(rows, dtype=torch.int64).to(ctx.device)
# ... 323 lines not shown
    if not OPT.bf16_twin_only:
        return n
    for h in buffers:
        if h.t16 is not None and h.writers and not any(reads_twin(r) for r in h.readers):
            for w in h.writers:
                if isinstance(w, L.InFwdDesc):
                    w.out_bf16 = None
                else:
                    w.dy_bf16 = None
            h.t16 = None
            n += 1
            continue
        if h.t16 is None or h.pinned or not h.readers or not h.writers or not all(reads_twin(r) for r in h.readers):
            continue
        if not all(isinstance(w, L.InFwdDesc) or (isinstance(w, L.InBwdDesc) and w.norm) for w in h.writers):
            continue
        for w in h.writers:
            if isinstance(w, L.InFwdDesc):
                w.out = None
            else:
                w.dy = None
            n += 1
        h.fp32_dead = True
    return n


def emit_in_bwd(plan: Plan, ctx: Ctx, *, g: Optional[Halo], g_fold=False, g2: Optional[Halo] = None, a: Optional[Halo] = None,
                act=L.ACT_NONE, slope=0.2, y: Optional[Halo] = None, stats=None, norm=True, dy: Halo, gsum: Optional[Halo] = None,
                dbias: Optional[torch.Tensor] = None, ws=None, shape=None, sums_only: bool = False, pre_sums: int = 0):
    B, H, W, Cc = shape
    d = L.InBwdDesc()
    if g is not None:
        assert g.H == H and g.W == W and g.C == Cc
        d.g, d.g_hp, d.g_wp, d.g_pad, d.g_fold = g.ptr_any(), g.hp, g.wp, g.pad, (1 if g_fold else 0)
        d.g_bf16 = 1 if g.is16 else 0
    if g2 is not None:
        assert g2.pad == 0
        d.g2 = g2.ptr
    d.act, d.slope = act, slope
    d.norm = 1 if norm else 0
    if y is not None:
        d.y, d.y_bf16 = y.ptr_any(), (1 if y.is16 else 0)
    if norm:
        d.mean, d.rstd = stats[0].data_ptr(), stats[1].data_ptr()
    if norm or dbias is not None:
        d.ws, d.ws_elems = ws.data_ptr(), ws.numel()
    d.B, d.H, d.W, d.C = B, H, W, Cc
    assert not sums_only or norm
    d.dy, d.d_hp, d.d_wp, d.d_pad = (None if sums_only else dy.operand_ptr()), dy.hp, dy.wp, dy.pad
    if dy.t16 is not None and not sums_only:
        d.dy_bf16 = dy.t16.data_ptr()
        dy.writers.append(d)
    if gsum is not None:
        d.gsum_out = gsum.ptr
    if pre_sums:
        assert norm and (gsum is not None or (g is not None and not g_fold and g2 is None))
        d.sums_chunks = pre_sums
    if dbias is not None:
        d.dbias = dbias.data_ptr()
    ctx.keep.append(d)
    plan.add("nirgan_instnorm_bwd", C.byref(d))
    return d


class _Scratch:

    def __init__(self, ctx: Ctx):
        self.ctx, self.n = ctx, 0
        self.t: Optional[torch.Tensor] = None

    def want(self, B, H, W, Cc):
        self.n = max(self.n, int(L.backend().nirgan_instnorm_ws_elems(B, H, W, Cc)))

    def get(self) -> torch.Tensor:
        if self.t is None or self.t.numel() < self.n:
            self.t = self.ctx.zeros(max(self.n, 4))
            self.ctx.keep.append(self.t)
        return self.t


class ConvIN:

    def __init__(self, eng, name, kind, inp: Halo, weight, bias, *, k, s, p, cout, norm=True, act=L.ACT_RELU,
                 out_pad=0, out_border=L.BORDER_KEEP, residual: Optional[Halo] = None, cin_real=None, keep_z=False):
        self.eng, self.name, self.kind = eng, name, kind
        self.inp, self.weight, self.bias = inp, weight, bias
        self.k, self.s, self.p, self.cout = k, s, p, cout
        self.norm, self.act, self.residual = norm, act, residual
        self.cin = inp.C if kind != "rowpacked" else cin_real
        ctx = eng.ctx
        if kind == "convT":
            self.OH, self.OW = inp.H * 2, inp.W * 2
        else:
            self.OH, self.OW = G.conv_out(inp.H, k, s, p), G.conv_out(inp.W, k, s, p)
        assert inp.pad >= (p if kind != "convT" else 1), (name, inp.pad, p)
        B = inp.B
        phase_px = self.OH * self.OW // (4 if kind == "convT" else 1)
        y16 = (ctx.precision == 1 and norm and OPT.bf16_y and OPT.epilogue_stats and cout % 4 == 0 and phase_px % 128 == 0
               and self.OH * self.OW >= min(OPT.epilogue_min_pixels, OPT.epilogue_min_pixels_bf16) and one_pass_tiles(B * phase_px, cout))
        self.y = Halo(ctx, B, self.OH, self.OW, cout, 0, bf16=y16)
        self.out = Halo(ctx, B, self.OH, self.OW, cout, out_pad, twin=True)
        eng.__dict__.setdefault("twinned", []).append(self.out)
        self.out_border = out_border
        self.stats = (ctx.zeros(B, cout), ctx.zeros(B, cout)) if norm else None
        eng.scratch.want(B, self.OH, self.OW, cout)
        self.keep_z = keep_z

    def emit_fwd(self, plan: Plan, pack: Plan):
        eng, ctx, inp = self.eng, self.eng.ctx, self.inp
        k, s, p = self.k, self.s, self.p
        pre = None
        if self.kind == "conv" and wino_applicable(ctx, inp, k, s, p, self.cout, self.OH, self.OW):
            keep = bool(getattr(eng, "need_backward", False))
            prod = getattr(self, "producer", None)
            xn = (prod.y, prod.stats, prod.act) if prod is not None and getattr(prod, "defer_apply", False) else None
            self.wino6 = True
            sws = None
            if self.norm and OPT.epilogue_stats:
                T = _w6_tiles(inp.B, self.OH, self.OW, wino6_variant(k))
                if not hasattr(ctx, "wino6_pool_stats"):
                    ctx.wino6_pool_stats = SplitPool(ctx)
                sws = ctx.wino6_pool_stats.get(T * 4 * self.cout)
                pre = (T // inp.B, self.bias, sws)
            self.wino_fwd = emit_wino6(plan, pack, ctx, inp, self.weight, self.bias, self.y, H=self.OH, W=self.OW, cin=inp.C,
                                       cout=self.cout, own_V=keep, x_norm=xn, r=k, stats_ws=sws)
            self.wino_fwd_keeps_V = keep
        elif self.kind == "conv":
            taps = G.conv_fwd_taps(k, inp.C)
            w = eng.weights.packed(pack, self.weight, G.conv_fwd_pack(self.cout, inp.C, k))
            cd = emit_conv(plan, ctx, inp, taps, w, self.bias, self.y, N=self.cout, OH=self.OH, OW=self.OW,
                           in_stride=s, in_oh=inp.pad - p, in_ow=inp.pad - p)
            if self.norm:
                pre = attach_conv_stats(ctx, [cd], self.bias)
            self._y_fallback(pre, [cd])
        elif (self.kind == "rowpacked" and s == 1 and ctx.precision == 0 and OPT.split3 and OPT.pair_pixels and self.cout == 64
              and (k + 1) * inp.C == 32 and self.OW % 2 == 0 and inp.wp % 2 == 0 and (inp.pad - p) % 2 == 0 and not self.y.is16):
            cs = inp.C
            w = eng.weights.packed_pair(pack, self.weight, [G.conv_rowpacked_pair_pack(self.cout, self.cin, k, cs, q) for q in (0, 1)])
            b2 = eng.weights.doubled(pack, self.bias) if self.bias is not None else None
            cd = emit_conv(plan, ctx, inp, G.Taps(list(range(k)), [0] * k, (k + 1) * cs), w, b2, self.y, N=2 * self.cout, OH=self.OH, OW=self.OW // 2,
                           in_oh=inp.pad - p, in_ow=(inp.pad - p) // 2, in_hw=(inp.hp, inp.wp // 2), in_cs=2 * cs,
                           out_hw=(self.y.hp, self.y.wp // 2), out_cs=2 * self.cout, out_span=2)
            if self.norm:
                pre = attach_conv_stats(ctx, [cd], self.bias)
        elif self.kind == "rowpacked":
            taps = G.conv_rowpacked_taps(k, inp.C)
            w = eng.weights.packed(pack, self.weight, G.conv_rowpacked_pack(self.cout, self.cin, k, inp.C))
            cd = emit_conv(plan, ctx, inp, taps, w, self.bias, self.y, N=self.cout, OH=self.OH, OW=self.OW,
                           in_stride=s, in_oh=inp.pad - p, in_ow=inp.pad - p)
            if self.norm:
                pre = attach_conv_stats(ctx, [cd], self.bias)
            self._y_fallback(pre, [cd])
        else:
            descs = None
            phases = G.convT_fwd_phases(inp.H, inp.W, k, p)
            if want_phase_pairs(ctx, phases, inp.C, self.cout, self.y):
                descs = emit_phase_pairs(eng, pack, ctx, inp, phases, lambda hw: G.convT_fwd_pack(inp.C, self.cout, k, hw), self.weight,
                                         self.bias, self.y, N=self.cout, in_off=inp.pad - 1, out_off=0)
            for ph in (phases if descs is None else []):
                descs = descs or []
                taps = G.Taps(ph.dh, ph.dw, inp.C)
                w = eng.weights.packed(pack, self.weight, G.convT_fwd_pack(inp.C, self.cout, k, ph.taps_hw))
                descs.append(emit_conv(None, ctx, inp, taps, w, self.bias, self.y, N=self.cout, OH=ph.n_h, OW=ph.n_w,
                                       in_oh=ph.in_oh + inp.pad - 1, in_ow=ph.in_ow + inp.pad - 1,
                                       out_stride=2, out_oh=ph.out_oh, out_ow=ph.out_ow))
            if self.norm:
                pre = attach_conv_stats(ctx, descs, self.bias)
            self._y_fallback(pre, descs)
            emit_conv_group(plan, ctx, descs)
        emit_in_fwd(plan, ctx, self.y, self.out, norm=self.norm, act=(L.ACT_NONE if self.keep_z else self.act),
                    residual=self.residual, border=self.out_border, stats=self.stats, ws=(pre[2] if pre is not None else eng.scratch.get()),
                    stats_only=getattr(self, "defer_apply", False), pre_stats=(pre[:2] if pre is not None else None))

    def _y_fallback(self, pre, descs):
        if self.y.is16 and pre is None:
            self.y = Halo(self.eng.ctx, self.inp.B, self.OH, self.OW, self.cout, 0)
            for d in descs:
                d.out, d.out_bf16 = self.y.ptr, 0

    def alloc_bwd(self, need_dgrad: bool):
        ctx, k = self.eng.ctx, self.k
        if self.kind == "convT":
            zpad = 1
        elif self.s == 1:
            zpad = k - 1 if need_dgrad else 0
        else:
            zpad = 1 if need_dgrad else 0
        self.dy = Halo(ctx, self.inp.B, self.OH, self.OW, self.cout, zpad, twin=True)
        self.eng.__dict__.setdefault("twinned", []).append(self.dy)

    def emit_bwd(self, plan: Plan, pack: Plan, *, g: Optional[Halo], g_fold=False, g2: Optional[Halo] = None,
                 gsum: Optional[Halo] = None, gw: Optional[torch.Tensor], gb: Optional[torch.Tensor], dgrad_out: Optional[Halo],
                 mask: Optional[Halo] = None, act=None):
        eng, ctx, inp = self.eng, self.eng.ctx, self.inp
        k, s, p = self.k, self.s, self.p
        act = self.act if act is None else act
        dy = self.dy
        w6_bwd = (self.kind == "conv" and s == 1 and gw is not None and dgrad_out is not None and dgrad_out.pad == p and dy.pad == k - 1
                  and wino_dgrad_applicable(ctx, k, s, dgrad_out, self.cout, inp.C) and inp.C > 64
                  and inp.pad == 1 and p == 1 and self.cout % 128 == 0)
        fuse_dy = (w6_bwd and k == 3 and self.norm and dy.t16 is None and OPT.fuse_dy_norm and wino6_variant(3) == 6
                   and act in (L.ACT_NONE, L.ACT_RELU, L.ACT_LRELU))
        pre_sums, ws = 0, eng.scratch.get()
        od = getattr(g, "w6_out_desc", None) if g is not None else None
        if od is not None and od.r == 6 and g_fold and self.norm and g.pad == 1 and dy.t16 is None and OPT.fuse_inbwd:
            mo = _w6_geo(od.r if od.r else 3)[0]
            Hp, Wp = od.H, od.W
            if (Hp == self.OH + 2 and Wp == self.OW + 2 and od.K == self.cout and od.B == inp.B and min(Hp, Wp) >= 6
                    and (Hp - 3) // mo == (Hp - 1) // mo and (Wp - 3) // mo == (Wp - 1) // mo):
                chunks = (-(-Hp // mo)) * (-(-Wp // mo))
                if gsum is None:
                    key = ("inbwd_gz", inp.B, self.OH, self.OW, self.cout)
                    pool = ctx.__dict__.setdefault("inbwd_pool", {})
                    if key not in pool:
                        pool[key] = Halo(ctx, inp.B, self.OH, self.OW, self.cout, 0)
                    gsum = pool[key]
                if not hasattr(ctx, "inbwd_part"):
                    ctx.inbwd_part = SplitPool(ctx)
                ws = ctx.inbwd_part.get(inp.B * chunks * 2 * self.cout + inp.B * 2 * self.cout)
                od.fuse_y, od.fuse_mean, od.fuse_rstd = self.y.ptr, self.stats[0].data_ptr(), self.stats[1].data_ptr()
                od.fuse_g2 = g2.ptr if g2 is not None else None
                od.fuse_gz, od.fuse_part, od.fuse_part_elems = gsum.ptr, ws.data_ptr(), ws.numel()
                od.fuse_act, od.fuse_slope = act, 0.2
                pre_sums = chunks
        cds = getattr(g, "conv_out_descs", None) if g is not None else None
        if (cds and not pre_sums and self.norm and not g_fold and g2 is None and gsum is None and self.cout % 4 == 0
                and act in (L.ACT_NONE, L.ACT_RELU, L.ACT_LRELU) and OPT.fuse_inbwd
                and all(c.ksplit <= 1 and (c.OH * c.OW) % 128 == 0 and channels_of(c) == self.cout and not c.bias for c in cds)
                and sum(c.OH * c.OW * max(1, c.out_span) for c in cds) == self.OH * self.OW
                and self.OH * self.OW >= (OPT.epilogue_min_pixels if ctx.precision == 0 else min(OPT.epilogue_min_pixels, OPT.epilogue_min_pixels_bf16))):
            chunks = sum(c.OH * c.OW // 128 * max(1, c.out_span) for c in cds)
            if not hasattr(ctx, "inbwd_part"):
                ctx.inbwd_part = SplitPool(ctx)
            ws = ctx.inbwd_part.get(inp.B * chunks * 2 * self.cout + inp.B * 2 * self.cout)
            first = 0
            for c in cds:
                c.fuse_y, c.fuse_mean, c.fuse_rstd = self.y.ptr_any(), self.stats[0].data_ptr(), self.stats[1].data_ptr()
                c.fuse_y_bf16 = 1 if self.y.is16 else 0
                c.fuse_h, c.fuse_w = self.OH, self.OW
                c.fuse_oh, c.fuse_ow = c.out_oh - g.pad, c.out_ow - g.pad
                c.fuse_act, c.fuse_slope = act, 0.2
                c.fuse_part, c.fuse_part_elems, c.fuse_chunk0, c.fuse_chunks = ws.data_ptr(), ws.numel(), first, chunks
                first += c.OH * c.OW // 128 * max(1, c.out_span)
            pre_sums = chunks
        nd = emit_in_bwd(plan, ctx, g=g, g_fold=g_fold, g2=g2, act=act,
                         y=self.y, stats=self.stats, norm=self.norm, dy=self.dy, gsum=gsum,
                         dbias=(None if self.norm else gb),
                         ws=ws,
                         shape=(inp.B, self.OH, self.OW, self.cout), pre_sums=pre_sums, sums_only=fuse_dy)
        if w6_bwd:
            wd6 = emit_wino6(None, pack, ctx, dy, self.weight, None, _FullExtent(dgrad_out), H=dgrad_out.hp, W=dgrad_out.wp,
                             cin=self.cout, cout=inp.C, flip=True, r=k)
            keepV = getattr(self, "wino_fwd_keeps_V", False) and getattr(self, "wino6", False)
            emit_wino6_backward(plan, ctx, dy, inp, gw, OH=self.OH, OW=self.OW, cin=inp.C, cout=self.cout, slabs_pool=eng.slabs,
                                dgrad=wd6, V_fwd=(self.wino_fwd if keepV else None), r=k, norm_desc=(nd if fuse_dy else None))
            if k == 3:
                dgrad_out.w6_out_desc = wd6
            return
        if self.kind == "conv" and s == 1 and gw is not None and dgrad_out is not None:
            assert dgrad_out.H == inp.H and dgrad_out.pad == p and dy.pad == k - 1
            hw = [(kh, kw) for kh in range(k) for kw in range(k)]
            wd = eng.weights.packed(pack, self.weight, G.conv_dgrad_pack(self.cout, inp.C, k, hw))
            cdesc = emit_conv(None, ctx, dy, G.conv_dgrad_s1_taps(k, self.cout), wd, None, dgrad_out, N=inp.C,
                              OH=dgrad_out.hp, OW=dgrad_out.wp)
            emit_wgrad(plan, ctx, dy, inp, G.conv_fwd_taps(k, inp.C), G.conv_fwd_pack(self.cout, inp.C, k), gw,
                       N=self.cout, OH=self.OH, OW=self.OW, p_oh=dy.pad, p_ow=dy.pad, q_stride=s,
                       q_oh=inp.pad - p, q_ow=inp.pad - p, slabs_pool=eng.slabs, pair_with=cdesc)
            return
        if gw is None:
            pass
        elif self.kind == "conv":
            emit_wgrad(plan, ctx, dy, inp, G.conv_fwd_taps(k, inp.C), G.conv_fwd_pack(self.cout, inp.C, k), gw,
                       N=self.cout, OH=self.OH, OW=self.OW, p_oh=dy.pad, p_ow=dy.pad, q_stride=s,
                       q_oh=inp.pad - p, q_ow=inp.pad - p, slabs_pool=eng.slabs)
        elif self.kind == "rowpacked" and s == 1 and emit_wgrad_pixel_pairs(plan, ctx, dy, inp, gw, k=k, p=p, cin=self.cin, cout=self.cout,
                                                                            OH=self.OH, OW=self.OW):
            pass
        elif self.kind == "rowpacked":
            emit_wgrad(plan, ctx, dy, inp, G.conv_rowpacked_taps(k, inp.C), G.conv_rowpacked_pack(self.cout, self.cin, k, inp.C), gw,
                       N=self.cout, OH=self.OH, OW=self.OW, p_oh=dy.pad, p_ow=dy.pad, q_stride=s,
                       q_oh=inp.pad - p, q_ow=inp.pad - p, slabs_pool=eng.slabs)
        else:
            emit_wgrad(plan, ctx, inp, dy, G.convT_dgrad_taps(k, self.cout), G.convT_dgrad_pack(inp.C, self.cout, k), gw,
                       N=inp.C, OH=inp.H, OW=inp.W, p_oh=inp.pad, p_ow=inp.pad, q_stride=2,
                       q_oh=dy.pad - p, q_ow=dy.pad - p, slabs_pool=eng.slabs)
        if dgrad_out is None:
            return
        if self.kind == "conv" and s == 1:
            assert dgrad_out.H == inp.H and dgrad_out.pad == p and dy.pad == k - 1
            if gw is None and wino_dgrad_applicable(ctx, k, s, dgrad_out, self.cout, inp.C) and inp.C > 64:
                emit_wino6(plan, pack, ctx, dy, self.weight, None, _FullExtent(dgrad_out), H=dgrad_out.hp, W=dgrad_out.wp,
                           cin=self.cout, cout=inp.C, flip=True, r=k)
                return
            taps = G.conv_dgrad_s1_taps(k, self.cout)
            hw = [(kh, kw) for kh in range(k) for kw in range(k)]
            w = eng.weights.packed(pack, self.weight, G.conv_dgrad_pack(self.cout, inp.C, k, hw))
            emit_conv(plan, ctx, dy, taps, w, None, dgrad_out, N=inp.C, OH=dgrad_out.hp, OW=dgrad_out.wp)
        elif self.kind in ("conv", "rowpacked") and s == 2:
            assert dgrad_out.H == inp.H and dy.pad == 1
            cin_buf = inp.C
            descs = None
            phases = G.conv_dgrad_s2_phases(inp.H, inp.W, k, p)
            if self.kind == "conv" and want_phase_pairs(ctx, phases, self.cout, inp.C, dgrad_out):
                descs = emit_phase_pairs(eng, pack, ctx, dy, phases, lambda hw: G.conv_dgrad_pack(self.cout, inp.C, k, hw), self.weight, None,
                                         dgrad_out, N=inp.C, in_off=0, out_off=dgrad_out.pad)
            for ph in (phases if descs is None else []):
                descs = descs or []
                if self.kind == "conv":
                    spec = G.conv_dgrad_pack(self.cout, inp.C, k, ph.taps_hw)
                else:
                    spec = G.conv_dgrad_pack(self.cout, self.cin, k, ph.taps_hw)
                    cin_buf = self.cin
                w = eng.weights.packed(pack, self.weight, spec)
                descs.append(emit_conv(None, ctx, dy, G.Taps(ph.dh, ph.dw, self.cout), w, None, dgrad_out, N=cin_buf,
                                       OH=ph.n_h, OW=ph.n_w, in_oh=ph.in_oh, in_ow=ph.in_ow, out_stride=2,
                                       out_oh=ph.out_oh + dgrad_out.pad, out_ow=ph.out_ow + dgrad_out.pad))
            emit_conv_group(plan, ctx, descs)
            dgrad_out.conv_out_descs = descs
        elif self.kind == "convT":
            assert dgrad_out.H == inp.H and dy.pad == 1
            w = eng.weights.packed(pack, self.weight, G.convT_dgrad_pack(inp.C, self.cout, k))
            cd = emit_conv(plan, ctx, dy, G.convT_dgrad_taps(k, self.cout), w, None, dgrad_out, N=inp.C, OH=inp.H, OW=inp.W,
                           in_stride=2, in_oh=dy.pad - p, in_ow=dy.pad - p, out_oh=dgrad_out.pad, out_ow=dgrad_out.pad)
            dgrad_out.conv_out_descs = [cd]
        else:
            raise NotImplementedError(self.kind)


# ... 84 lines not shown
```

### nir-gan_amd/nirgan_hip/lib.py

```python
from __future__ import annotations

import ctypes as C
import os

_HERE = os.path.dirname(os.path.abspath(__file__))
LIB_PATH = os.path.join(os.path.dirname(_HERE), "lib", "libnirgan_hip.so")

MAX_TAPS = 16
ACT_NONE, ACT_RELU, ACT_LRELU, ACT_TANH = 0, 1, 2, 3
BORDER_KEEP, BORDER_REFLECT = 0, 1
OP_CONV, OP_WGRAD, OP_IN_FWD, OP_IN_BWD = 1, 2, 3, 4

fp = C.c_void_p
i32, i64, f32 = C.c_int, C.c_int64, C.c_float


class ConvDesc(C.Structure):
    _fields_ = [("inp", fp), ("in_elems", i64), ("in_hp", i32), ("in_wp", i32), ("in_cs", i32),
                ("run", i32), ("in_stride", i32), ("in_oh", i32), ("in_ow", i32), ("ntaps", i32),
                ("tap_dh", i32 * MAX_TAPS), ("tap_dw", i32 * MAX_TAPS),
                ("w", fp), ("w_elems", i64), ("bias", fp),
                ("out", fp), ("out_elems", i64), ("out_hp", i32), ("out_wp", i32), ("out_cs", i32),
                ("out_stride", i32), ("out_oh", i32), ("out_ow", i32),
                ("B", i32), ("OH", i32), ("OW", i32), ("N", i32), ("zero_page", fp),
                ("ksplit", i32), ("split_ws", fp), ("split_ws_elems", i64), ("precision", i32), ("w_bf16", i32), ("in_bf16", i32),
                ("stats_ws", fp), ("stats_ws_elems", i64), ("stats_chunk0", i32), ("stats_chunks", i32),
                ("fuse_y", fp), ("fuse_mean", fp), ("fuse_rstd", fp), ("fuse_h", i32), ("fuse_w", i32), ("fuse_oh", i32), ("fuse_ow", i32),
                ("fuse_act", i32), ("fuse_slope", f32), ("fuse_part", fp), ("fuse_part_elems", i64), ("fuse_chunk0", i32), ("fuse_chunks", i32),
                ("out_bf16", i32), ("fuse_y_bf16", i32), ("algo", i32), ("w_x3", fp), ("w_x3_plane", i64), ("out_span", i32)]


class WgradDesc(C.Structure):
    _fields_ = [("p", fp), ("p_elems", i64), ("p_hp", i32), ("p_wp", i32), ("p_cs", i32), ("p_oh", i32), ("p_ow", i32),
                ("q", fp), ("q_elems", i64), ("q_hp", i32), ("q_wp", i32), ("q_cs", i32), ("q_stride", i32),
                ("q_oh", i32), ("q_ow", i32), ("run", i32), ("ntaps", i32),
                ("tap_dh", i32 * MAX_TAPS), ("tap_dw", i32 * MAX_TAPS),
                ("B", i32), ("OH", i32), ("OW", i32), ("N", i32),
                ("slabs", fp), ("slab_elems", i64), ("nsplit", i32), ("rows_per_split", i32), ("zero_page", fp),
                ("precision", i32), ("nplanes", i32), ("p_plane", i64), ("q_plane", i64), ("pq_bf16", i32), ("algo", i32)]


class InFwdDesc(C.Structure):
    _fields_ = [("y", fp), ("B", i32), ("H", i32), ("W", i32), ("C", i32), ("norm", i32), ("eps", f32),
                ("mean", fp), ("rstd", fp), ("act", i32), ("slope", f32),
                ("residual", fp), ("r_hp", i32), ("r_wp", i32), ("r_pad", i32),
                ("out", fp), ("o_hp", i32), ("o_wp", i32), ("o_pad", i32), ("border", i32),
                ("ws", fp), ("ws_elems", i64), ("out_bf16", fp), ("stats_chunks", i32), ("stats_shift", fp), ("y_bf16", i32)]


class InBwdDesc(C.Structure):
    _fields_ = [("g", fp), ("g_hp", i32), ("g_wp", i32), ("g_pad", i32), ("g_fold", i32), ("g2", fp),
                ("a", fp), ("a_hp", i32), ("a_wp", i32), ("a_pad", i32), ("act", i32), ("slope", f32),
                ("y", fp), ("mean", fp), ("rstd", fp), ("norm", i32),
                ("B", i32), ("H", i32), ("W", i32), ("C", i32),
                ("dy", fp), ("d_hp", i32), ("d_wp", i32), ("d_pad", i32),
                ("gsum_out", fp), ("dbias", fp), ("ws", fp), ("ws_elems", i64), ("dy_bf16", fp), ("sums_chunks", i32), ("y_bf16", i32), ("g_bf16", i32)]


class ChanDgradDesc(C.Structure):
    _fields_ = [("dy", fp), ("dy_hp", i32), ("dy_wp", i32), ("dy_pad", i32), ("C", i32),
                ("w", fp), ("cin", i32), ("k", i32), ("stride", i32), ("pad", i32), ("channel", i32),
                ("B", i32), ("H", i32), ("W", i32), ("out", fp)]


class TapGatherDesc(C.Structure):
    _fields_ = [("q", fp), ("q_hp", i32), ("q_wp", i32), ("q_cs", i32), ("ntaps", i32),
                ("tap_dh", i32 * 64), ("tap_dw", i32 * 64), ("bias", fp), ("act", i32),
                ("B", i32), ("OH", i32), ("OW", i32), ("crop", i32), ("dst", fp)]


class TapScatterDesc(C.Structure):
    _fields_ = [("dout", fp), ("out", fp), ("act", i32), ("B", i32), ("OH", i32), ("OW", i32), ("crop", i32),
                ("ntaps", i32), ("tap_dh", i32 * 64), ("tap_dw", i32 * 64),
                ("dq", fp), ("q_hp", i32), ("q_wp", i32), ("q_cs", i32), ("dbias", fp)]


GAN_VANILLA, GAN_WGANGP = 1, 2
GAN_MODES = {"vanilla": GAN_VANILLA, "wgangp": GAN_WGANGP}

PIX_LOSS_WS_ELEMS = 8192


class PixLossDesc(C.Structure):
    _fields_ = [("rgb", fp), ("nir", fp), ("pred", fp), ("B", i32), ("H", i32), ("W", i32),
                ("w_l1", f32), ("w_ndvi", f32), ("w_ndwi", f32), ("w_gndvi", f32), ("w_savi", f32),
                ("w_msavi", f32), ("w_evi", f32), ("criterion", i32), ("log_all", i32),
                ("extra", fp), ("extra_cs", i32), ("extra_c", i32), ("extra_scale", f32),
                ("sums", fp), ("grad_pred", fp), ("ws", fp), ("ws_elems", i64)]


PIXMLP_TILE = 32


class PixMlpDesc(C.Structure):
    _fields_ = [("rgb", fp), ("nir", fp), ("dpred", fp), ("B", i32), ("H", i32), ("W", i32), ("hidden", i32),
                ("params", fp), ("grads", fp), ("pred", fp), ("loss_out", fp), ("ws", fp), ("ws_elems", i64)]


class InjectFwdDesc(C.Structure):
    _fields_ = [("z", fp), ("e", fp), ("scale", fp), ("style", i32), ("B", i32), ("H", i32), ("W", i32), ("C", i32),
                ("out", fp), ("o_hp", i32), ("o_wp", i32), ("o_pad", i32)]


class InjectBwdDesc(C.Structure):
    _fields_ = [("g", fp), ("a", fp), ("a_hp", i32), ("a_wp", i32), ("a_pad", i32), ("z", fp), ("e", fp),
                ("scale", fp), ("style", i32), ("B", i32), ("H", i32), ("W", i32), ("C", i32),
                ("dz", fp), ("de", fp), ("dscale", fp), ("ws", fp), ("ws_elems", i64)]


class MetricsDesc(C.Structure):
    _fields_ = [("pred", fp), ("target", fp), ("planes", i32), ("H", i32), ("W", i32),
                ("window", i32), ("sigma", f32), ("max_val", f32), ("eps", f32),
# ... 131 lines not shown
    "nirgan_conv_wgrad_pair_kernel_name": (C.c_char_p, [C.POINTER(ConvDesc), C.POINTER(WgradDesc)]),
    "nirgan_reduce_rows": (i32, [fp, i32, i32, i32, fp, fp, i64, i32, i32, fp]),
    "nirgan_reduce_rows_part": (i32, [fp, i32, i32, i32, i32, i32, fp, fp, i64, i32, i32, fp]),
    "nirgan_reduce_rows_batch": (i32, [fp, i32, i32, fp]),
    "nirgan_pack_rows": (i32, [fp, i64, i32, fp, fp, i32, i32, fp]),
    "nirgan_pack_rows_bf16": (i32, [fp, i64, i32, fp, fp, i32, i32, fp]),
    "nirgan_pack_rows_batch": (i32, [fp, i32, i32, fp]),
    "nirgan_split3": (i32, [fp, fp, i64, i64, fp]),
    "nirgan_location_encoder": (i32, [C.POINTER(LocEncDesc), fp]),
    "nirgan_tile_count": (i64, [i32, i32, i32, i32, i32]),
    "nirgan_tile_gather": (i32, [fp, i32, i32, i32, i32, i32, i32, i32, i32, fp, fp]),
    "nirgan_tile_scatter": (i32, [fp, i32, i32, i32, i32, i32, i32, i32, i32, fp, fp]),
    "nirgan_tile_count_ov": (i64, [i32, i32, i32, i32, i32, i32]),
    "nirgan_tile_gather_ov": (i32, [C.POINTER(TileBlendDesc), fp]),
    "nirgan_tile_blend": (i32, [C.POINTER(TileBlendDesc), fp]),
    "nirgan_tile_views_expand": (i32, [C.POINTER(TileViewsDesc), fp]),
    "nirgan_tile_views_merge": (i32, [C.POINTER(TileViewsDesc), fp]),
    "nirgan_point_regions_ws_bytes": (i64, [i32, i32]),
    "nirgan_region_boxes": (i32, [C.POINTER(PointRegionsDesc), fp]),
    "nirgan_point_regions": (i32, [C.POINTER(PointRegionsDesc), fp]),
    "nirgan_raster_lookup": (i32, [C.POINTER(RasterLookupDesc), fp]),
    "nirgan_wino6_tiles": (i64, [i32, i32, i32]),
    "nirgan_wino6_tiles_r": (i64, [i32, i32, i32, i32]),
    "nirgan_wino6_weights": (i32, [fp, i32, i32, i32, fp, fp]),
    "nirgan_wino6_weights_r": (i32, [fp, i32, i32, i32, i32, fp, fp]),
    "nirgan_wino6_weights_x3": (i32, [fp, i32, i32, i32, i32, fp, fp, fp]),
    "nirgan_wino6_weights_batch": (i32, [fp, i32, i32, fp]),
    "nirgan_wino6_input": (i32, [C.POINTER(Wino6Desc), fp]),
    "nirgan_wino6_input_norm": (i32, [C.POINTER(Wino6Desc), fp, fp, fp, i32, f32, fp]),
    "nirgan_wino6_input_dy_norm": (i32, [C.POINTER(Wino6Desc), C.POINTER(WinoDyDesc), C.POINTER(InBwdDesc), fp]),
    "nirgan_wino6_gemm": (i32, [C.POINTER(Wino6Desc), fp]),
    "nirgan_wino6_gemm_wgrad_pair": (i32, [C.POINTER(Wino6Desc), C.POINTER(WgradDesc), fp]),
    "nirgan_wino6_gemm_kernel_name": (C.c_char_p, [C.POINTER(Wino6Desc)]),
    "nirgan_wino6_pair_kernel_name": (C.c_char_p, [C.POINTER(Wino6Desc), C.POINTER(WgradDesc)]),
    "nirgan_wino6_output": (i32, [C.POINTER(Wino6Desc), fp]),
    "nirgan_wino6_conv3x3": (i32, [C.POINTER(Wino6Desc), fp]),
    "nirgan_wino6_dy": (i32, [C.POINTER(WinoDyDesc), fp]),
    "nirgan_wino6_input_dy": (i32, [C.POINTER(Wino6Desc), C.POINTER(WinoDyDesc), fp]),
    "nirgan_wino6_wgrad_finish": (i32, [fp, i32, i32, i32, fp, i32, fp]),
    "nirgan_wino6_wgrad_finish_r": (i32, [fp, i32, i32, i32, i32, fp, i32, fp]),
    "nirgan_wino6_wgrad_finish_batch": (i32, [fp, fp, i32, i32, i32, i32, i32, i32, fp]),
    "nirgan_hist_match_ws_bytes": (i64, [i32, i32]),
    "nirgan_hist_match": (i32, [C.POINTER(HistMatchDesc), fp]),
    "nirgan_image_metrics_ws_elems": (i64, [i32, i32, i32]),
    "nirgan_image_metrics": (i32, [C.POINTER(MetricsDesc), fp]),
    "nirgan_tile_metrics_ws_elems": (i64, [i32, i32, i32]),
    "nirgan_tile_metrics": (i32, [C.POINTER(TileMetricsDesc), fp]),
    "nirgan_window_stats": (i32, [C.POINTER(WindowStatsDesc), fp]),
    "nirgan_val_panel_ws_bytes": (i64, [i32, i32, i32]),
    "nirgan_val_panel": (i32, [C.POINTER(ValPanelDesc), fp]),
    "nirgan_class_metrics_ws_elems": (i64, [i32, i32, i32, i32]),
    "nirgan_class_metrics": (i32, [C.POINTER(ClassMetricsDesc), fp]),
    "nirgan_ssim_loss_ws_elems": (i64, [i32, i32, i32, i32]),
    "nirgan_ssim_loss": (i32, [C.POINTER(SsimLossDesc), fp]),
    "nirgan_emd_loss_ws_bytes": (i64, [i32, i64, i32]),
    "nirgan_emd_loss": (i32, [C.POINTER(EmdLossDesc), fp]),
    "nirgan_instnorm_ws_elems": (i64, [i32, i32, i32, i32]),
    "nirgan_instnorm_fwd": (i32, [C.POINTER(InFwdDesc), fp]),
    "nirgan_instnorm_bwd": (i32, [C.POINTER(InBwdDesc), fp]),
    "nirgan_nchw_to_halo": (i32, [fp, i32, i32, i32, i32, fp, i32, i32, i32, i32, i32, fp]),
    "nirgan_conv_channel_dgrad": (i32, [C.POINTER(ChanDgradDesc), fp]),
    "nirgan_tap_gather": (i32, [C.POINTER(TapGatherDesc), fp]),
    "nirgan_tap_scatter": (i32, [C.POINTER(TapScatterDesc), fp]),
    "nirgan_endconv_dz_elems": (i64, [i32, i32, i32]),
    "nirgan_endconv_ws_elems": (i64, [i32, i32, i32]),
    "nirgan_endconv_fwd": (i32, [C.POINTER(EndConvDesc), fp]),
    "nirgan_endconv_dz": (i32, [C.POINTER(EndConvDesc), fp]),
    "nirgan_endconv_dgrad": (i32, [C.POINTER(EndConvDesc), fp]),
    "nirgan_endconv_wgrad": (i32, [C.POINTER(EndConvDesc), fp]),
    "nirgan_lsgan": (i32, [fp, i64, f32, f32, fp, fp, fp]),
    "nirgan_gan_loss": (i32, [fp, i64, i32, f32, f32, fp, fp, fp]),
    "nirgan_pix_loss": (i32, [C.POINTER(PixLossDesc), fp]),
    "nirgan_pixmlp_fwd": (i32, [C.POINTER(PixMlpDesc), fp]),
    "nirgan_pixmlp_train": (i32, [C.POINTER(PixMlpDesc), fp]),
    "nirgan_pixmlp_ws_elems": (i64, [i32, i32, i32, i32]),
    "nirgan_adam": (i32, [fp, fp, fp, fp, i64, f32, f32, f32, f32, i32, fp]),
    "nirgan_bilinear_fwd": (i32, [fp, i32, i32, i32, fp, i32, i32, fp]),
    "nirgan_bilinear_bwd": (i32, [fp, i32, i32, i32, fp, i32, i32, fp]),
    "nirgan_inject_fwd": (i32, [C.POINTER(InjectFwdDesc), fp]),
    "nirgan_inject_bwd": (i32, [C.POINTER(InjectBwdDesc), fp]),
    "nirgan_param_scale_fwd": (i32, [fp, fp, fp, i64, fp]),
    "nirgan_param_scale_bwd": (i32, [fp, fp, fp, fp, fp, fp, i64, i64, fp]),
    "nirgan_colsum": (i32, [fp, i64, i32, fp, i32, fp]),
    "nirgan_fill": (i32, [fp, i64, f32, fp]),
    "nirgan_axpy": (i32, [fp, fp, i64, f32, fp]),
    "nirgan_run_plan": (i32, [C.POINTER(PlanEntry), i32, fp]),
}


class _CLib:

    is_emulator = False

    def __init__(self, path: str):
        if not os.path.exists(path):
            raise ImportError(
                f"{path} not found: build the HIP extension first (python __graft_entry__.py). "
                "The NIR-GAN MI355X path has no CPU fallback.")
        import torch
        self._dll = C.CDLL(path)
        for name, (res, args) in PROTOTYPES.items():
            fn = getattr(self._dll, name)
            fn.restype = res
            fn.argtypes = args
            setattr(self, name, fn)


_real = _CLib(LIB_PATH)
_backend = _real


def check_exports() -> None:
    for name in PROTOTYPES:
        getattr(_real, name)
    assert _real.nirgan_version() >= 100


def backend():
    return _backend


def set_backend(obj) -> None:
    global _backend
    _backend = _real if obj is None else obj


def is_emulated() -> bool:
    return _backend is not _real


def check(rc: int, what: str = "") -> None:
    if rc != 0:
        msg = _backend.nirgan_last_error()
        if isinstance(msg, bytes):
            msg = msg.decode()
        raise RuntimeError(f"libnirgan_hip {what} failed ({rc}): {msg}")


def call(name: str, *args) -> None:
    check(getattr(_backend, name)(*args), name)
```

### nir-gan_amd/nirgan_hip/nets.py

```python
from __future__ import annotations

import ctypes as C
from typing import Dict, Optional

import torch

from . import geometry as G
from . import lib as L
from .options import OPT
from .engine import (ConvIN, Ctx, Halo, Plan, SlabPool, TapPlaneConv, Weights, _Scratch, drop_dead_fp32_stores, emit_conv, grad_halo,
                     emit_deferred_reduce_rows, emit_w6_deferred_finishes, emit_wgrad, wino_applicable)


def generator_layout(n_blocks: int) -> dict:
    up0 = 10 + n_blocks
    return {"first": 1, "down": [4, 7], "blocks": list(range(10, 10 + n_blocks)), "up": [up0, up0 + 3], "last": up0 + 7}


class _Engine:
    def __init__(self, device, precision="fp32"):
        self.ctx = Ctx(device, precision)
        self.weights = Weights(self.ctx)
        self.slabs = SlabPool(self.ctx)
        self.scratch = _Scratch(self.ctx)
# ... 165 lines not shown
            self.pc_ws = ctx.zeros(1024)
            gpc = gr["post_correction_param"]
            b.add("nirgan_fill", gpc.data_ptr(), 1, 0.0)
            b.add("nirgan_param_scale_bwd", self.dpred.data_ptr(), self.pred_raw.data_ptr(), self.params["post_correction_param"].data_ptr(),
                  self.last.dout.data_ptr(), gpc.data_ptr(), self.pc_ws.data_ptr(), self.pc_ws.numel(), self.dpred.numel())
        for layer in [self.L1]:
            layer.alloc_bwd(need_dgrad=False)
        for layer in [self.L2, self.L3, self.U1, self.U2] + [c for _, c1, c2 in self.blocks for c in (c1, c2)]:
            layer.alloc_bwd(need_dgrad=True)
        il = lay["last"]
        b.add("nirgan_fill", GW(il, "bias").data_ptr(), 1, 0.0)
        self.last.emit_bwd(b, pk, GW(il), GW(il, "bias"))
        i0, i1 = lay["up"]
        g_u1 = grad_halo(ctx, B, self.U1.OH, self.U1.OW, self.U1.cout, 0)
        self.U2.emit_bwd(b, pk, g=self.last.gin, g_fold=True, gw=GW(i1), gb=GW(i1, "bias"), dgrad_out=g_u1)
        c4, H3, W3 = self.L3.cout, self.L3.OH, self.L3.OW
        g_top = Halo(ctx, B, H3, W3, c4, 0)
        self.U1.emit_bwd(b, pk, g=g_u1, gw=GW(i0), gb=GW(i0, "bias"), dgrad_out=g_top)
        g_in, g_fold, g_skip = g_top, False, None
        dense = [Halo(ctx, B, H3, W3, c4, 0), Halo(ctx, B, H3, W3, c4, 0)] if self.blocks else []
        flip = 0
        ctx.w6_deferred = []
        for j in range(len(self.blocks) - 1, -1, -1):
            i, c1, c2 = self.blocks[j]
            gq = grad_halo(ctx, B, H3, W3, c4, 1)
            gp = grad_halo(ctx, B, H3, W3, c4, 1)
            if g_skip is None:
                gsum, skip_next = None, g_in
            else:
                gsum, skip_next = dense[flip], dense[flip]
                flip ^= 1
            c2.emit_bwd(b, pk, g=g_in, g_fold=g_fold, g2=g_skip, gsum=gsum, gw=GW(i, "conv_block.5.weight"),
                        gb=GW(i, "conv_block.5.bias"), dgrad_out=gq, act=L.ACT_NONE)
            c1.emit_bwd(b, pk, g=gq, g_fold=True, gw=GW(i, "conv_block.1.weight"), gb=GW(i, "conv_block.1.bias"), dgrad_out=gp)
            g_in, g_fold, g_skip = gp, True, skip_next
        emit_w6_deferred_finishes(b, ctx)
        emit_deferred_reduce_rows(b, ctx, last=False)
        first_tail = f"model.{lay['blocks'][0]}.conv_block.1.weight" if self.blocks else f"model.{i0}.weight"
        self.bwd_tail = (len(b.ops), first_tail, f"model.{il}.bias")
        g_a2 = grad_halo(ctx, B, self.L2.OH, self.L2.OW, self.L2.cout, 0, phases=4) if self.inject is None else Halo(ctx, B, self.L2.OH, self.L2.OW, self.L2.cout, 0)
        self.L3.emit_bwd(b, pk, g=g_in, g_fold=g_fold, g2=g_skip, gw=GW(7), gb=GW(7, "bias"), dgrad_out=g_a2)
        g_a1 = grad_halo(ctx, B, self.L1.OH, self.L1.OW, self.L1.cout, 0, phases=4)
        if self.inject is None:
            self.L2.emit_bwd(b, pk, g=g_a2, gw=GW(4), gb=GW(4, "bias"), dgrad_out=g_a1)
        else:
            dz2 = self._emit_inject_bwd(b, g_a2)
            self.L2.emit_bwd(b, pk, g=dz2, gw=GW(4), gb=GW(4, "bias"), dgrad_out=g_a1, act=L.ACT_NONE)
        emit_deferred_reduce_rows(b, ctx, last=False)
        self.bwd_mid = (len(b.ops), "model.1.weight", "model.1.bias")
        self.L1.emit_bwd(b, pk, g=g_a1, gw=GW(1), gb=GW(1, "bias"), dgrad_out=None)
        emit_deferred_reduce_rows(b, ctx)

    def forward(self, rgb: torch.Tensor, embeds: Optional[torch.Tensor] = None, version: int = 0) -> torch.Tensor:
        self.refresh_weights(version)
        self.rgb_in.copy_(rgb)
        if self.inject is not None:
            self.emb_in.t.view(self.B, 256).copy_(embeds)
        self.fwd.run()
        return self.pred

    def backward(self, dpred: Optional[torch.Tensor], version: int = 0) -> None:
        self.refresh_weights(version, backward=True)
        if dpred is not None:
            self.dpred.copy_(dpred)
        self.bwd.run()


class DiscriminatorEngine(_Engine):

    def __init__(self, params: Dict[str, torch.Tensor], grads: Optional[Dict[str, torch.Tensor]], B: int, H: int, W: int,
                 need_backward: bool = True, precision="fp32"):
        dev = params["model.0.weight"].device
        super().__init__(dev, precision)
        ctx = self.ctx
        self.params, self.grads, self.B, self.H, self.W = params, grads, B, H, W
        ndf, in_nc = params["model.0.weight"].shape[0], params["model.0.weight"].shape[1]
        assert in_nc == 4, "PatchGAN input is cat(rgb, nir) = 4 channels on this path"

        def P(i, what):
            return params[f"model.{i}.{what}"]

        self.x_in = ctx.zeros(B, 4, H, W)
        self.x4 = Halo(ctx, B, H, W, 4, 1)
        self.C1 = ConvIN(self, "c1", "rowpacked", self.x4, P(0, "weight"), P(0, "bias"), k=4, s=2, p=1, cout=ndf, norm=False,
                         act=L.ACT_LRELU, out_pad=1, cin_real=4)
        self.C2 = ConvIN(self, "c2", "conv", self.C1.out, P(2, "weight"), P(2, "bias"), k=4, s=2, p=1, cout=2 * ndf, act=L.ACT_LRELU, out_pad=1)
        self.C3 = ConvIN(self, "c3", "conv", self.C2.out, P(5, "weight"), P(5, "bias"), k=4, s=2, p=1, cout=4 * ndf, act=L.ACT_LRELU, out_pad=1)
        self.C4 = ConvIN(self, "c4", "conv", self.C3.out, P(8, "weight"), P(8, "bias"), k=4, s=1, p=1, cout=8 * ndf, act=L.ACT_LRELU, out_pad=1)
        self.C5 = TapPlaneConv(self, "c5", self.C4.out, P(11, "weight"), P(11, "bias"), k=4, p=1)
        self.out = self.C5.dst
        f, pk = self.fwd, self.pack_fwd
        self.in_plan = Plan(ctx)
        self.in_plan.add("nirgan_nchw_to_halo", self.x_in.data_ptr(), B, 4, H, W, self.x4.ptr, 4, 0, 0, 1, L.BORDER_KEEP)
        for layer in (self.C1, self.C2, self.C3, self.C4, self.C5):
            layer.emit_fwd(f, pk)
        self._part_plans: dict = {}
        if need_backward:
            self._build_backward()
        drop_dead_fp32_stores(getattr(self, "twinned", []))

    def _build_backward(self):
        ctx, b, pk, gr, B = self.ctx, self.bwd, self.pack_bwd, self.grads, self.B
        self.C5.alloc_bwd()
        self.dout = self.C5.dout
        for layer in (self.C1, self.C2, self.C3, self.C4):
            layer.alloc_bwd(need_dgrad=True)
        self.g3p = grad_halo(ctx, B, self.C3.OH, self.C3.OW, self.C3.cout, 1)
        self.g2 = grad_halo(ctx, B, self.C2.OH, self.C2.OW, self.C2.cout, 0, phases=4)
        self.g1 = grad_halo(ctx, B, self.C1.OH, self.C1.OW, self.C1.cout, 0, phases=4)
        self.gx4 = Halo(ctx, B, self.H, self.W, 4, 0)
        self.gpred = ctx.zeros(B, self.H, self.W)
        self.bwd_frozen = Plan(ctx)
        self.bwd_pred = Plan(ctx)
        for plan, mode in ((b, "train"), (self.bwd_frozen, "input"), (self.bwd_pred, "pred")):
            frozen = mode != "train"

            def GW(i, what="weight"):
                return None if frozen else gr[f"model.{i}.{what}"]
            if not frozen:
                for k in ("model.0.bias", "model.11.bias"):
                    plan.add("nirgan_fill", gr[k].data_ptr(), gr[k].numel(), 0.0)
                ctx.rr_deferred = [] if OPT.batch_reduce else None
            self.C5.emit_bwd(plan, pk, GW(11), GW(11, "bias"))
            self.C4.emit_bwd(plan, pk, g=self.C5.gin, g_fold=False, gw=GW(8), gb=GW(8, "bias"), dgrad_out=self.g3p)
            if not frozen:
                emit_deferred_reduce_rows(plan, ctx, last=False)
                self.bwd_tail = (len(plan.ops), "model.8.weight", "model.11.bias")
            self.C3.emit_bwd(plan, pk, g=self.g3p, g_fold=False, gw=GW(5), gb=GW(5, "bias"), dgrad_out=self.g2)
            self.C2.emit_bwd(plan, pk, g=self.g2, gw=GW(2), gb=GW(2, "bias"), dgrad_out=self.g1)
            if not frozen:
                emit_deferred_reduce_rows(plan, ctx, last=False)
                self.bwd_mid = (len(plan.ops), "model.0.weight", "model.0.bias")
            self.C1.emit_bwd(plan, pk, g=self.g1, gw=GW(0), gb=GW(0, "bias"), dgrad_out=self.gx4 if mode == "input" else None)
            if not frozen:
                emit_deferred_reduce_rows(plan, ctx)
            if mode == "pred":
                d = L.ChanDgradDesc()
                dy, w = self.C1.dy, self.params["model.0.weight"]
                d.dy, d.dy_hp, d.dy_wp, d.dy_pad, d.C = dy.ptr, dy.hp, dy.wp, dy.pad, dy.C
                d.w, d.cin, d.k, d.stride, d.pad, d.channel = w.data_ptr(), 4, 4, 2, 1, 3
                d.B, d.H, d.W, d.out = B, self.H, self.W, self.gpred.data_ptr()
                ctx.keep.append(d)
                plan.add("nirgan_conv_channel_dgrad", C.byref(d))

    def input_plan(self, parts) -> Plan:
        key = tuple((t.data_ptr(), t.shape[0], t.shape[1], b0, c0) for t, b0, c0 in parts)
        if key not in self._part_plans:
            pl = Plan(self.ctx)
            for t, b0, c0 in parts:
                nb, cs = t.shape[0], t.shape[1]
                assert t.is_contiguous() and t.shape[2] == self.H and t.shape[3] == self.W and b0 + nb <= self.B
                dst = self.x4.ptr + b0 * self.x4.hp * self.x4.wp * 4 * 4
                pl.add("nirgan_nchw_to_halo", t.data_ptr(), nb, cs, self.H, self.W, dst, 4, c0, 0, 1, L.BORDER_KEEP)
            self._part_plans[key] = pl
        return self._part_plans[key]

    def forward(self, x: Optional[torch.Tensor] = None, parts=None, version: int = 0) -> torch.Tensor:
        self.refresh_weights(version)
        if parts is not None:
            self.input_plan(parts).run()
        else:
            self.x_in.copy_(x)
            self.in_plan.run()
        self.fwd.run()
        return self.out

    def backward(self, dout: Optional[torch.Tensor], frozen: bool = False, version: int = 0, pred_only: bool = False) -> Optional[torch.Tensor]:
        self.refresh_weights(version, backward=True)
# ... 11 lines not shown
```

### nir-gan_amd/nirgan_hip/options.py

```python
from __future__ import annotations

import os


class Options:
    w6_gemm_algo: int = 0
    wgrad_algo: int = 0
    w6_pair: bool = True
    winograd: str = "f6"
    epilogue_stats: bool = True
    fuse_inbwd: bool = True
    epilogue_min_pixels: int = 16384
    epilogue_min_pixels_bf16: int = 1024
    fuse_dy_norm: bool = True
    dp_buckets: bool = True
    bf16_y: bool = True
    bf16_g: bool = True
    bf16_store_min_tiles: int = 100
    bf16_twin_only: bool = True
    fold_apply: bool = True
    tile256: bool = True
    batch_reduce: bool = True
    wgrad_target: int = 512
    split3: bool = True
    split3_wino: bool = True
    pair_phases: bool = True
    pair_pixels: bool = True
    x3_r4: bool = True
    endconv_direct: bool = True

    def reset(self):
        for k, v in vars(Options).items():
            if not k.startswith("_") and not callable(v):
                setattr(self, k, v)


    def update_from(self, text: str):
        for item in filter(None, (t.strip() for t in text.split(","))):
            k, _, v = item.partition("=")
            if not hasattr(Options, k) or k.startswith("_"):
                raise ValueError(f"NIRGAN_OPTIONS: unknown option '{k}'")
            cur = getattr(Options, k)
            setattr(self, k, (v.lower() in ("1", "true", "yes", "on")) if isinstance(cur, bool) else type(cur)(v))


OPT = Options()
if os.environ.get("NIRGAN_OPTIONS"):
    OPT.update_from(os.environ["NIRGAN_OPTIONS"])
```

Measured before the change: 1122 tiles/s.

## Fuse LeakyReLU mask into dgrad epilogue for un-normalized discriminator first layer

Adds a no-norm mode to the fused instance-norm-backward epilogue: the dgrad conv multiplies its output by the activation derivative read from the post-activation tensor and accumulates bias-gradient partials, which a new strided colsum reduces. It also adds an optional activation-in-conv-epilogue path, off by default, that skips storing the pre-activation y. Together these aim to remove the separate activation-backward / bias-gradient pass (and optionally the y store) for the PatchGAN first layer. The cost is extra epilogue work, a partial-sum workspace, and more routing conditions in the register-fed x3 kernel.

```diff
diff --git a/include/nirgan_hip.h b/include/nirgan_hip.h
--- a/include/nirgan_hip.h
+++ b/include/nirgan_hip.h
@@ -49,6 +49,7 @@
     int out_bf16, fuse_y_bf16;
     int algo;
     const void* w_x3; int64_t w_x3_plane;
+    int out_act; float out_slope;
     int out_span;
 } nirgan_conv_desc;
 #define NIRGAN_CONV_TILE128 1
@@ -423,6 +424,7 @@
 int nirgan_inject_bwd(const nirgan_inject_bwd_desc* d, void* stream);
 
 int nirgan_colsum(const float* x, int64_t rows, int cols, float* out, int accumulate, void* stream);
+int nirgan_colsum_ld(const float* x, int64_t rows, int cols, int64_t ld, float* out, int accumulate, void* stream);
 
 int nirgan_param_scale_fwd(const float* x, const float* param, float* out, int64_t n, void* stream);
 int nirgan_param_scale_bwd(const float* gout, const float* x, const float* param, float* gx, float* dparam, float* ws, int64_t ws_elems,
diff --git a/nir-gan_amd/csrc/elementwise.hip b/nir-gan_amd/csrc/elementwise.hip
--- a/nir-gan_amd/csrc/elementwise.hip
+++ b/nir-gan_amd/csrc/elementwise.hip
@@ -171,19 +171,19 @@
     if (tid == 0 && p.dscale) p.ws[blockIdx.x] = (red[0] + red[1]) + (red[2] + red[3]);
 }
 
-__global__ __launch_bounds__(1024) void colsum_kernel(const float* __restrict__ x, int64_t rows, int cols, float* __restrict__ out, int accumulate) {
+__global__ __launch_bounds__(1024) void colsum_kernel(const float* __restrict__ x, int64_t rows, int cols, int64_t ld, float* __restrict__ out, int accumulate) {
     __shared__ float red[16][64];
     const int cl = threadIdx.x & 63, c = blockIdx.x * 64 + cl, rl = threadIdx.x >> 6;
     float s0 = 0.f, s1 = 0.f, s2 = 0.f, s3 = 0.f;
     if (c < cols) {
         int64_t r = rl;
         for (; r + 48 < rows; r += 64) {
-            s0 += x[r * cols + c];
-            s1 += x[(r + 16) * cols + c];
-            s2 += x[(r + 32) * cols + c];
-            s3 += x[(r + 48) * cols + c];
-        }
-        for (; r < rows; r += 16) s0 += x[r * cols + c];
+            s0 += x[r * ld + c];
+            s1 += x[(r + 16) * ld + c];
+            s2 += x[(r + 32) * ld + c];
+            s3 += x[(r + 48) * ld + c];
+        }
+        for (; r < rows; r += 16) s0 += x[r * ld + c];
     }
     red[rl][cl] = (s0 + s1) + (s2 + s3);
     __syncthreads();
@@ -322,8 +322,14 @@
 
 extern "C" int nirgan_colsum(const float* x, int64_t rows, int cols, float* out, int accumulate, void* stream) {
     NG_REQUIRE(x && out && rows > 0 && cols > 0, "colsum: bad arguments");
-    hipLaunchKernelGGL(colsum_kernel, dim3((cols + 63) / 64), dim3(1024), 0, static_cast<hipStream_t>(stream), x, rows, cols, out, accumulate);
+    hipLaunchKernelGGL(colsum_kernel, dim3((cols + 63) / 64), dim3(1024), 0, static_cast<hipStream_t>(stream), x, rows, cols, int64_t(cols), out, accumulate);
     return nirgan_check_launch("colsum");
+}
+
+extern "C" int nirgan_colsum_ld(const float* x, int64_t rows, int cols, int64_t ld, float* out, int accumulate, void* stream) {
+    NG_REQUIRE(x && out && rows > 0 && cols > 0 && ld >= cols, "colsum_ld: bad arguments");
+    hipLaunchKernelGGL(colsum_kernel, dim3((cols + 63) / 64), dim3(1024), 0, static_cast<hipStream_t>(stream), x, rows, cols, ld, out, accumulate);
+    return nirgan_check_launch("colsum_ld");
 }
 
 extern "C" int nirgan_fill(float* dst, int64_t n, float value, void* stream) {
diff --git a/nir-gan_amd/csrc/igemm_conv.hip b/nir-gan_amd/csrc/igemm_conv.hip
--- a/nir-gan_amd/csrc/igemm_conv.hip
+++ b/nir-gan_amd/csrc/igemm_conv.hip
@@ -153,7 +153,7 @@
 ng::X3Kernel ng::conv_x3_route(const ng::ConvParams* ps, const int n, const int bn) {
     bool reg_fed = true, gen = false, stats = false;
     for (int i = 0; i < n; ++i) {
-        reg_fed = reg_fed && ng::conv_x3r_ok(ps[i], bn);
+        reg_fed = reg_fed && ng::conv_x3r_ok(ps[i], bn) && !(ps[i].f_y != nullptr && ps[i].f_mean == nullptr);
         gen = gen || ng::conv_x3r_generic(ps[i]);
         stats = stats || ng::conv_x3r_stats(ps[i]);
     }
diff --git a/nir-gan_amd/csrc/igemm_tiles.h b/nir-gan_amd/csrc/igemm_tiles.h
--- a/nir-gan_amd/csrc/igemm_tiles.h
+++ b/nir-gan_amd/csrc/igemm_tiles.h
@@ -81,6 +81,7 @@
     long long w3_plane;
     int ch;
     long long out_elems;
+    int o_act; float o_slope;
 };
 
 
@@ -457,19 +458,33 @@
         int oh = r0 / p.OW, ow = r0 - oh * p.OW;
         const int OH = p.OHW / p.OW;
         const bool fused = p.f_y != nullptr;
+        const bool nonorm = fused && p.f_mean == nullptr;
         const int fb = m0 / p.OHW;
         fW fm = {}, fr = {}, s1 = {}, s2 = {};
-        if (fused && n < p.N) {
+        if (fused && !nonorm && n < p.N) {
             fm = *reinterpret_cast<const fW*>(p.f_mean + size_t(fb) * p.N + n);
             fr = *reinterpret_cast<const fW*>(p.f_rstd + size_t(fb) * p.N + n);
         }
         const float fneg = p.f_act == NIRGAN_ACT_RELU ? 0.f : (p.f_act == NIRGAN_ACT_LRELU ? p.f_slope : 1.f);
+        const bool oact = p.o_act != NIRGAN_ACT_NONE && !to_ws;
+        const bool orelu = p.o_act == NIRGAN_ACT_RELU;
+        const float oneg = p.o_act == NIRGAN_ACT_LRELU ? p.o_slope : 1.f;
 #pragma unroll 4
         for (int row = row0; row < BM; row += RPP) {
             if (m < p.M && n < p.N) {
                 const float* src = reinterpret_cast<const float*>(row < 64 ? st0 : st1) + (row & 63) * BN + chunk * W;
                 fW v = *reinterpret_cast<const fW*>(src);
                 v += bv;
+                if (oact) {
+#pragma unroll
+                    for (int j = 0; j < W; ++j) v[j] = v[j] > 0.f ? v[j] : (orelu ? 0.f : v[j] * oneg);
+                }
+                fW y4 = {};
+                if (nonorm) {
+                    y4 = *reinterpret_cast<const fW*>(p.f_y + (size_t(b) * p.f_img + size_t(oh * p.out_stride) * p.f_row + size_t(ow * p.out_stride) * p.N + p.f_org + n));
+#pragma unroll
+                    for (int j = 0; j < W; ++j) v[j] = y4[j] > 0.f ? v[j] : v[j] * fneg;
+                }
                 const int oidx = b * p.out_img + oh * p.out_stride * p.out_row + ow * p.out_stride * p.out_cs + p.out_org + n;
                 float* dst = to_ws ? p.split_ws + ((size_t(ksp) * p.M + m) * p.N + n) : p_out + oidx;
                 if constexpr (W == 8) {
@@ -483,9 +498,10 @@
                     for (int j = 0; j < W; ++j)
                         if (n + j < p.N) dst[j] = v[j];
                 }
-                if (fused) {
+                if (nonorm) {
+                    s1 += v;
+                } else if (fused) {
                     const size_t yidx = size_t(b) * p.f_img + size_t(oh * p.out_stride) * p.f_row + size_t(ow * p.out_stride) * p.N + p.f_org + n;
-                    fW y4;
                     if (p.f_y16) y4 = __builtin_convertvector(*reinterpret_cast<const bW*>(reinterpret_cast<const unsigned short*>(p.f_y) + yidx), fW);
                     else y4 = *reinterpret_cast<const fW*>(p.f_y + yidx);
                     const fW z = (y4 - fm) * fr;
@@ -1257,7 +1273,10 @@
     p.f_img = p.f_row = p.f_org = p.f_chunk0 = p.f_cps = 0; p.f_act = NIRGAN_ACT_NONE; p.f_slope = 0.f;
     if (d->fuse_y != nullptr) {
         NG_REQUIRE(d->ksplit <= 1 && p.OHW % 128 == 0 && d->N % 4 == 0 && d->bias == nullptr, "conv: the fused instance-norm backward sums need OH*OW %% 128 == 0, N %% 4 == 0, no split-K and no bias (OH*OW=%d N=%d)", p.OHW, d->N);
-        NG_REQUIRE(d->fuse_mean && d->fuse_rstd && d->fuse_part && ng_aligned16(d->fuse_y) && ng_aligned16(d->fuse_mean) && ng_aligned16(d->fuse_rstd) && ng_aligned16(d->fuse_part), "conv: fuse_mean / fuse_rstd / fuse_part missing or misaligned");
+        const bool nonorm = d->fuse_mean == nullptr && d->fuse_rstd == nullptr;
+        NG_REQUIRE(!nonorm || (!d->out_bf16 && !d->fuse_y_bf16 && ch % 4 == 0 && (d->precision == 0 || d->precision == 3)),
+                   "conv: fuse_y without fuse_mean / fuse_rstd needs fp32 tensors, precision 0 or 3 and channels %% 4 == 0");
+        NG_REQUIRE((nonorm || (d->fuse_mean && d->fuse_rstd)) && d->fuse_part && ng_aligned16(d->fuse_y) && ng_aligned16(d->fuse_mean) && ng_aligned16(d->fuse_rstd) && ng_aligned16(d->fuse_part), "conv: fuse_mean / fuse_rstd / fuse_part missing or misaligned");
         NG_REQUIRE(d->fuse_oh >= 0 && d->fuse_ow >= 0 && (d->OH - 1) * d->out_stride + d->fuse_oh < d->fuse_h && (d->OW - 1) * d->out_stride + d->fuse_ow + span - 1 < d->fuse_w, "conv: fused window out of y's %d x %d extent", d->fuse_h, d->fuse_w);
         NG_REQUIRE(int64_t(d->B) * d->fuse_h * d->fuse_w * ch < (int64_t(1) << 31), "conv: fuse_y must be < 2^31 floats");
         NG_REQUIRE(d->fuse_chunk0 >= 0 && d->fuse_chunk0 + p.OHW / 128 * span <= d->fuse_chunks, "conv: fuse_chunk0 + OH*OW/128 (x out_span) exceeds fuse_chunks");
@@ -1266,6 +1285,13 @@
         p.f_y = d->fuse_y; p.f_mean = d->fuse_mean; p.f_rstd = d->fuse_rstd; p.f_part = d->fuse_part;
         p.f_row = d->fuse_w * ch; p.f_img = d->fuse_h * p.f_row; p.f_org = d->fuse_oh * p.f_row + d->fuse_ow * ch;
         p.f_act = d->fuse_act; p.f_slope = d->fuse_slope; p.f_chunk0 = d->fuse_chunk0; p.f_cps = d->fuse_chunks;
+    }
+    p.o_act = NIRGAN_ACT_NONE; p.o_slope = 0.f;
+    if (d->out_act != NIRGAN_ACT_NONE) {
+        NG_REQUIRE(d->out_act == NIRGAN_ACT_RELU || d->out_act == NIRGAN_ACT_LRELU, "conv: out_act=%d (NIRGAN_ACT_NONE, NIRGAN_ACT_RELU or NIRGAN_ACT_LRELU)", d->out_act);
+        NG_REQUIRE(d->ksplit <= 1 && d->stats_ws == nullptr && d->fuse_y == nullptr && !d->out_bf16 && span == 1 && d->precision == 0,
+                   "conv: out_act needs the fp32 store of the 128-row tile (precision 0; no split-K, stats_ws, fuse_y, out_bf16 or out_span)");
+        p.o_act = d->out_act; p.o_slope = d->out_slope;
     }
     if (d->ksplit > 1) {
         const int nk = d->ntaps * ((d->run + 31) / 32);
diff --git a/nir-gan_amd/csrc/igemm_x3.h b/nir-gan_amd/csrc/igemm_x3.h
--- a/nir-gan_amd/csrc/igemm_x3.h
+++ b/nir-gan_amd/csrc/igemm_x3.h
@@ -293,6 +293,7 @@
         const int sw_wr = ((lane >> 4) & SWM) << 4;
         float* const stg = reinterpret_cast<float*>(wave < 6 ? sA1 + wave * 8192 : sB1 + (wave - 6) * 8192);
         const bool fused = f_y != nullptr;
+        const bool nonorm = fused && p.f_mean == nullptr;
         const float fneg = p.f_act == NIRGAN_ACT_RELU ? 0.f : (p.f_act == NIRGAN_ACT_LRELU ? p.f_slope : 1.f);
         const int chunk = lane % LPR, lrow = lane / LPR;
         const int n = E.n0 + wc * CW + chunk * 4;
@@ -306,7 +307,7 @@
         const int fb = (mbase < pM ? mbase : pM - 1) / OHW;
         f32x4 fm = {0.f, 0.f, 0.f, 0.f}, fr = fm, s1 = fm, s2 = fm;
         const int nq = n >= pC ? 1 : 0, nc = n - nq * pC;
-        if (fused) {
+        if (fused && !nonorm) {
             fm = *reinterpret_cast<const f32x4*>(p.f_mean + size_t(fb) * pC + nc);
             fr = *reinterpret_cast<const f32x4*>(p.f_rstd + size_t(fb) * pC + nc);
         }
@@ -339,12 +340,18 @@
                     if (ok[pass]) {
                         f32x4 v = *reinterpret_cast<const f32x4*>(stg + (pass * RPP + lrow) * CW + ((chunk * 4) ^ ((((pass * RPP + lrow) >> 2) & SWM) << 4)));
                         v += bv;
+                        if (nonorm) {
+#pragma unroll
+                            for (int q = 0; q < 4; ++q) v[q] = yv[pass][q] > 0.f ? v[q] : v[q] * fneg;
+                        }
 #ifdef NG_X3_NT_STORES
                         __builtin_nontemporal_store(v, reinterpret_cast<f32x4*>(E.out + ooff[pass]));
 #else
                         *reinterpret_cast<f32x4*>(E.out + ooff[pass]) = v;
 #endif
-                        if (fused) {
+                        if (nonorm) {
+                            s1 += v;
+                        } else if (fused) {
                             const f32x4 z = (yv[pass] - fm) * fr;
 #pragma unroll
                             for (int q = 0; q < 4; ++q) {
diff --git a/nir-gan_amd/nirgan_hip/engine.py b/nir-gan_amd/nirgan_hip/engine.py
--- a/nir-gan_amd/nirgan_hip/engine.py
+++ b/nir-gan_amd/nirgan_hip/engine.py
@@ -294,6 +294,11 @@
         return 1
     k = max(1, min(8, 1024 // max(tiles, 1), nk // 16))
     return k if k > 1 else 1
+
+
+def conv_ksplit(M: int, N: int, ntaps: int, run: int) -> int:
+    tiles = -(-M // 128) * (-(-N // 128) if N > 64 else 1)
+    return choose_ksplit(tiles, ntaps * (-(-run // 32))) if N % 4 == 0 else 1
 
 
 def emit_conv(plan: Plan, ctx: Ctx, inp: Halo, taps: G.Taps, w: torch.Tensor, bias, out: Halo, *, N, OH, OW,
@@ -333,8 +338,7 @@
     ctx.keep.append(d)
     if plan is not None:
         M = inp.B * OH * OW
-        tiles = -(-M // 128) * (-(-N // 128) if N > 64 else 1)
-        ks = choose_ksplit(tiles, taps.n * (-(-taps.run // 32))) if (allow_split and N % 4 == 0) else 1
+        ks = conv_ksplit(M, N, taps.n, taps.run) if allow_split else 1
         if ks > 1:
             if not hasattr(ctx, "split_pool"):
                 ctx.split_pool = SplitPool(ctx)
@@ -824,7 +828,7 @@
 class ConvIN:
 
     def __init__(self, eng, name, kind, inp: Halo, weight, bias, *, k, s, p, cout, norm=True, act=L.ACT_RELU,
-                 out_pad=0, out_border=L.BORDER_KEEP, residual: Optional[Halo] = None, cin_real=None, keep_z=False):
+                 out_pad=0, out_border=L.BORDER_KEEP, residual: Optional[Halo] = None, cin_real=None, keep_z=False, y_unread=False):
         self.eng, self.name, self.kind = eng, name, kind
         self.inp, self.weight, self.bias = inp, weight, bias
         self.k, self.s, self.p, self.cout = k, s, p, cout
@@ -840,7 +844,14 @@
         phase_px = self.OH * self.OW // (4 if kind == "convT" else 1)
         y16 = (ctx.precision == 1 and norm and OPT.bf16_y and OPT.epilogue_stats and cout % 4 == 0 and phase_px % 128 == 0
                and self.OH * self.OW >= min(OPT.epilogue_min_pixels, OPT.epilogue_min_pixels_bf16) and one_pass_tiles(B * phase_px, cout))
-        self.y = Halo(ctx, B, self.OH, self.OW, cout, 0, bf16=y16)
+        run = inp.C if kind == "conv" else k * inp.C
+        self.act_in_conv = bool(
+            OPT.conv_act and y_unread and not L.is_emulated() and not norm and residual is None and act in (L.ACT_RELU, L.ACT_LRELU)
+            and out_border == L.BORDER_KEEP and ctx.precision == 0 and not keep_z and cout % 4 == 0
+            and (kind == "conv" or (kind == "rowpacked" and s != 1)) and not (OPT.split3 and run % 32 == 0)
+            and not (kind == "conv" and wino_applicable(ctx, inp, k, s, p, cout, self.OH, self.OW))
+            and conv_ksplit(B * self.OH * self.OW, cout, k * k if kind == "conv" else k, run) == 1)
+        self.y = None if self.act_in_conv else Halo(ctx, B, self.OH, self.OW, cout, 0, bf16=y16)
         self.out = Halo(ctx, B, self.OH, self.OW, cout, out_pad, twin=True)
         eng.__dict__.setdefault("twinned", []).append(self.out)
         self.out_border = out_border
@@ -870,6 +881,8 @@
         elif self.kind == "conv":
             taps = G.conv_fwd_taps(k, inp.C)
             w = eng.weights.packed(pack, self.weight, G.conv_fwd_pack(self.cout, inp.C, k))
+            if self.act_in_conv:
+                return self._emit_fwd_act(plan, taps, w)
             cd = emit_conv(plan, ctx, inp, taps, w, self.bias, self.y, N=self.cout, OH=self.OH, OW=self.OW,
                            in_stride=s, in_oh=inp.pad - p, in_ow=inp.pad - p)
             if self.norm:
@@ -888,6 +901,8 @@
         elif self.kind == "rowpacked":
             taps = G.conv_rowpacked_taps(k, inp.C)
             w = eng.weights.packed(pack, self.weight, G.conv_rowpacked_pack(self.cout, self.cin, k, inp.C))
+            if self.act_in_conv:
+                return self._emit_fwd_act(plan, taps, w)
             cd = emit_conv(plan, ctx, inp, taps, w, self.bias, self.y, N=self.cout, OH=self.OH, OW=self.OW,
                            in_stride=s, in_oh=inp.pad - p, in_ow=inp.pad - p)
             if self.norm:
@@ -913,6 +928,14 @@
         emit_in_fwd(plan, ctx, self.y, self.out, norm=self.norm, act=(L.ACT_NONE if self.keep_z else self.act),
                     residual=self.residual, border=self.out_border, stats=self.stats, ws=(pre[2] if pre is not None else eng.scratch.get()),
                     stats_only=getattr(self, "defer_apply", False), pre_stats=(pre[:2] if pre is not None else None))
+
+    def _emit_fwd_act(self, plan: Plan, taps: G.Taps, w):
+        inp, out = self.inp, self.out
+        cd = emit_conv(plan, self.eng.ctx, inp, taps, w, self.bias, out, N=self.cout, OH=self.OH, OW=self.OW, in_stride=self.s,
+                       in_oh=inp.pad - self.p, in_ow=inp.pad - self.p, out_oh=out.pad, out_ow=out.pad)
+        assert cd.ksplit <= 1 and cd.precision == 0 and not cd.out_bf16, (self.name, cd.ksplit, cd.precision)
+        cd.out_act, cd.out_slope = self.act, 0.2
+        return cd
 
     def _y_fallback(self, pre, descs):
         if self.y.is16 and pre is None:
@@ -985,7 +1008,33 @@
                 c.fuse_part, c.fuse_part_elems, c.fuse_chunk0, c.fuse_chunks = ws.data_ptr(), ws.numel(), first, chunks
                 first += c.OH * c.OW // 128 * max(1, c.out_span)
             pre_sums = chunks
-        nd = emit_in_bwd(plan, ctx, g=g, g_fold=g_fold, g2=g2, act=act,
+        masked = bool(
+            cds and not self.norm and OPT.dgrad_mask and OPT.fuse_inbwd and not L.is_emulated() and ctx.precision == 0 and not g_fold
+            and g2 is None and gsum is None and mask is None and self.cout % 4 == 0 and act in (L.ACT_RELU, L.ACT_LRELU)
+            and dy.t16 is None and not g.is16 and not self.keep_z
+            and all(c.ksplit <= 1 and (c.OH * c.OW) % 128 == 0 and channels_of(c) == self.cout and not c.bias and not c.out_bf16
+                    and c.precision in (0, 3) for c in cds)
+            and sum(c.OH * c.OW * max(1, c.out_span) for c in cds) == self.OH * self.OW)
+        if self.y is None and not masked:
+            raise RuntimeError(f"layer {self.name}: built without its pre-activation (y_unread), but this backward plan needs it")
+        if masked:
+            chunks = sum(c.OH * c.OW // 128 * max(1, c.out_span) for c in cds)
+            if not hasattr(ctx, "inbwd_part"):
+                ctx.inbwd_part = SplitPool(ctx)
+            part = ctx.inbwd_part.get(inp.B * chunks * 2 * self.cout)
+            out, first = self.out, 0
+            for c in cds:
+                oh, ow = c.out_oh - g.pad, c.out_ow - g.pad
+                c.out, c.out_elems, c.out_hp, c.out_wp = dy.ptr, dy.elems, dy.hp, dy.wp
+                c.out_oh, c.out_ow = oh + dy.pad, ow + dy.pad
+                c.fuse_y, c.fuse_mean, c.fuse_rstd, c.fuse_y_bf16 = out.ptr, None, None, 0
+                c.fuse_h, c.fuse_w, c.fuse_oh, c.fuse_ow = out.hp, out.wp, oh + out.pad, ow + out.pad
+                c.fuse_act, c.fuse_slope = act, 0.2
+                c.fuse_part, c.fuse_part_elems, c.fuse_chunk0, c.fuse_chunks = part.data_ptr(), part.numel(), first, chunks
+                first += c.OH * c.OW // 128 * max(1, c.out_span)
+            if gb is not None:
+                plan.add("nirgan_colsum_ld", part.data_ptr(), inp.B * chunks, self.cout, 2 * self.cout, gb.data_ptr(), 1)
+        nd = None if masked else emit_in_bwd(plan, ctx, g=g, g_fold=g_fold, g2=g2, act=act,
                          y=self.y, stats=self.stats, norm=self.norm, dy=self.dy, gsum=gsum,
                          dbias=(None if self.norm else gb),
                          ws=ws,
diff --git a/nir-gan_amd/nirgan_hip/lib.py b/nir-gan_amd/nirgan_hip/lib.py
--- a/nir-gan_amd/nirgan_hip/lib.py
+++ b/nir-gan_amd/nirgan_hip/lib.py
@@ -27,7 +27,8 @@
                 ("stats_ws", fp), ("stats_ws_elems", i64), ("stats_chunk0", i32), ("stats_chunks", i32),
                 ("fuse_y", fp), ("fuse_mean", fp), ("fuse_rstd", fp), ("fuse_h", i32), ("fuse_w", i32), ("fuse_oh", i32), ("fuse_ow", i32),
                 ("fuse_act", i32), ("fuse_slope", f32), ("fuse_part", fp), ("fuse_part_elems", i64), ("fuse_chunk0", i32), ("fuse_chunks", i32),
-                ("out_bf16", i32), ("fuse_y_bf16", i32), ("algo", i32), ("w_x3", fp), ("w_x3_plane", i64), ("out_span", i32)]
+                ("out_bf16", i32), ("fuse_y_bf16", i32), ("algo", i32), ("w_x3", fp), ("w_x3_plane", i64), ("out_act", i32), ("out_slope", f32),
+                ("out_span", i32)]
 
 
 class WgradDesc(C.Structure):
@@ -325,6 +326,7 @@
     "nirgan_param_scale_fwd": (i32, [fp, fp, fp, i64, fp]),
     "nirgan_param_scale_bwd": (i32, [fp, fp, fp, fp, fp, fp, i64, i64, fp]),
     "nirgan_colsum": (i32, [fp, i64, i32, fp, i32, fp]),
+    "nirgan_colsum_ld": (i32, [fp, i64, i32, i64, fp, i32, fp]),
     "nirgan_fill": (i32, [fp, i64, f32, fp]),
     "nirgan_axpy": (i32, [fp, fp, i64, f32, fp]),
     "nirgan_run_plan": (i32, [C.POINTER(PlanEntry), i32, fp]),
diff --git a/nir-gan_amd/nirgan_hip/nets.py b/nir-gan_amd/nirgan_hip/nets.py
--- a/nir-gan_amd/nirgan_hip/nets.py
+++ b/nir-gan_amd/nirgan_hip/nets.py
@@ -271,8 +271,11 @@
 
         self.x_in = ctx.zeros(B, 4, H, W)
         self.x4 = Halo(ctx, B, H, W, 4, 1)
+        h1, w1 = G.conv_out(H, 4, 2, 1), G.conv_out(W, 4, 2, 1)
+        c1_masked = (OPT.dgrad_mask and OPT.fuse_inbwd and ndf % 4 == 0 and ctx.precision == 0
+                     and all((ph.n_h * ph.n_w) % 128 == 0 for ph in G.conv_dgrad_s2_phases(h1, w1, 4, 1)))
         self.C1 = ConvIN(self, "c1", "rowpacked", self.x4, P(0, "weight"), P(0, "bias"), k=4, s=2, p=1, cout=ndf, norm=False,
-                         act=L.ACT_LRELU, out_pad=1, cin_real=4)
+                         act=L.ACT_LRELU, out_pad=1, cin_real=4, y_unread=(not need_backward or c1_masked))
         self.C2 = ConvIN(self, "c2", "conv", self.C1.out, P(2, "weight"), P(2, "bias"), k=4, s=2, p=1, cout=2 * ndf, act=L.ACT_LRELU, out_pad=1)
         self.C3 = ConvIN(self, "c3", "conv", self.C2.out, P(5, "weight"), P(5, "bias"), k=4, s=2, p=1, cout=4 * ndf, act=L.ACT_LRELU, out_pad=1)
         self.C4 = ConvIN(self, "c4", "conv", self.C3.out, P(8, "weight"), P(8, "bias"), k=4, s=1, p=1, cout=8 * ndf, act=L.ACT_LRELU, out_pad=1)
diff --git a/nir-gan_amd/nirgan_hip/options.py b/nir-gan_amd/nirgan_hip/options.py
--- a/nir-gan_amd/nirgan_hip/options.py
+++ b/nir-gan_amd/nirgan_hip/options.py
@@ -28,6 +28,8 @@
     pair_pixels: bool = True
     x3_r4: bool = True
     endconv_direct: bool = True
+    conv_act: bool = False
+    dgrad_mask: bool = True
 
     def reset(self):
         for k, v in vars(Options).items():
```

Measured after the change: 1128 tiles/s, median of 6. No clear change (+0.5%).
